# xiaoxiaokuye/CODLAD

Hardware: AMD Instinct MI355X
Metric: sampled all-atom structures/sec (100-step DDPM, PED) (higher is better)
Workload: dtype f32 as f16x3 split (each fp32 operand = fp16 hi + fp16 lo, 22-bit; 3 f16 MFMAs per product, fp32 accumulate); everything outside the contractions fp32; 1 GPU; cfg2: PED-shaped test set, 4 proteins L=46/87/92/129 x 10 frames x num_ensemble 10 = 400 structures per GPU, 100-step DDPM (mpnn_diffusion) + VQ(4096x3) + IC_Decoder N6 + ic_to_xyz; structures_rank0=400, nodes_rank0=35400, edges_rank0=2182800, ddpm_steps=100, parallelism=replicas x1

## Files before the change

### codlad_amd/_lib.py

```python
import ctypes as C
import os

import torch

_HERE = os.path.dirname(os.path.abspath(__file__))
ABI_VERSION = 15
LIB_PATH = os.environ.get("CODLAD_HIP_LIB") or os.path.join(_HERE, "libcodlad_hip.so")

P = C.c_void_p


class EncLayer(C.Structure):
    _fields_ = [(n, P) for n in ("W1e", "W2", "W3", "W11e", "W12", "W13", "W1a", "W1c", "W11a", "W11c")] + \
               [("Win", P * 4), ("Wout", P * 4)] + \
               [(n, P) for n in ("b1", "b2", "b3", "b11", "b12", "b13", "b_in", "b_out")]


class DecLayer(C.Structure):
    _fields_ = [(n, P) for n in ("W1e", "W2", "W3", "W1a", "W1v", "TS")] + \
               [("Win", P * 4), ("Wout", P * 4)] + \
               [(n, P) for n in ("b1", "b2", "b3", "b_in", "b_out")]


class EncLayerH(C.Structure):
    _fields_ = [(n, P) for n in ("W1e", "W2", "W3", "W11e", "W12", "W13", "W1a", "W1c", "W11a", "W11c")] + \
               [("Win", P * 4), ("Wout", P * 4)] + \
               [(n, P) for n in ("b1", "b2", "b3", "b11", "b12", "b13", "b_in", "b_out")] + \
               [(n, C.c_int) for n in ("e1", "e2", "e3", "e11", "e12", "e13", "e_in", "e_out")]


class DecLayerH(C.Structure):
    _fields_ = [(n, P) for n in ("W1e", "W2", "W3", "W1a", "W1v")] + [("Win", P * 4), ("Wout", P * 4)] + \
               [(n, P) for n in ("TS", "b1", "b2", "b3", "b_in", "b_out")] + \
               [(n, C.c_int) for n in ("e1", "e2", "e3", "e_in", "e_out")]


class DenoiserWeights(C.Structure):
    _fields_ = [(n, P) for n in ("freqs", "rbf_mu", "t_w0", "t_b0", "t_w2", "t_b2")] + \
               [("ada_w", P * 7), ("ada_b", P * 7)] + \
               [(n, P) for n in ("x_in_w", "x_in_b", "pos_w", "pos_b", "edge_wT", "norm_w", "norm_b",
                                 "We_wT", "We_b", "out_w", "out_b")] + \
               [("enc", EncLayer * 3), ("dec", DecLayer * 3), ("precision", C.c_int),
                ("enc_h", EncLayerH * 3), ("dec_h", DecLayerH * 3), ("self_condition", C.c_int), ("out_dim", C.c_int)]


class Workspace(C.Structure):
    _fields_ = [(n, P) for n in ("hV", "hVenc", "S", "PQ", "hE", "status", "tile_list")] + [("n_tiles", C.c_int32)]


class DecoderWeights(C.Structure):
    _fields_ = [("angle", C.c_int), ("map_out_w", P), ("map_out_b", P), ("res_embed", P)] + \
               [(n, P * 4) for n in ("inv0_w", "inv0_b", "inv1_w", "inv1_b", "dist_w", "dist_b",
                                     "dense1_w", "dense1_b", "dense3_w", "dense3_b")] + \
               [(n, P) for n in ("bb_dist", "sc_dist", "bb_ang1_w", "bb_ang1_b", "bb_ang3_w", "bb_ang3_b",
                                 "sc_angle_emb", "sc_ang1_w", "sc_ang1_b", "sc_ang3_w", "sc_ang3_b",
                                 "bb_tor1_w", "bb_tor1_b", "bb_tor3_w", "bb_tor3_b")] + \
               [(n, P * 4) for n in ("tor1_w", "tor1_b", "tor3_w", "tor3_b")] + \
               [(n, P) for n in ("fin1_w", "fin1_b", "fin3_w", "fin3_b")]


class TpConvArgs(C.Structure):
    _fields_ = [("ptr", P), ("snd", P), ("n_recv", C.c_int32), ("xyz_recv", P), ("xyz_snd", P), ("typ_recv", P),
                ("typ_snd", P), ("r_sign", C.c_float), ("smear_stop", C.c_float), ("emb0_w", P), ("emb0_b", P),
                ("emb3_w", P), ("emb3_b", P), ("emb_in", C.c_int32), ("h_recv", P), ("d_recv", C.c_int32), ("h_snd", P),
                ("d_snd", C.c_int32), ("attr_recv_first", C.c_int32), ("fc0_w", P), ("fc0_b", P), ("fc3_w", P),
                ("fc3_b", P), ("depth", C.c_int32), ("out", P), ("accumulate", C.c_int32), ("group", C.c_int32),
                ("packed", P)]


class XyzGroup(C.Structure):
    _fields_ = [("ca_full", P), ("ic", P), ("orders", P), ("slot_to_out", P), ("xyz_out", P),
                ("B", C.c_int32), ("L", C.c_int32), ("n_atoms", C.c_int32), ("first_row", C.c_int32)]


class MetricInputs(C.Structure):
    _fields_ = [("xyz_recon", P), ("xyz", P), ("n_atoms", C.c_int64),
                ("edge_list", P), ("n_edges", C.c_int64), ("clash_list", P), ("n_clash", C.c_int64),
                ("bb_NO_list", P), ("n_bb", C.c_int64), ("interaction_list", P), ("n_inter", C.c_int64),
                ("pi_pi_list", P), ("n_pipi", C.c_int64),
                ("ic", P), ("ic_recon", P), ("ic_mask", P), ("n_ic", C.c_int64)]


_SIGS = {
    "codlad_abi_version": (C.c_int, []),
    "codlad_probe_edge_launches": (C.c_int, [C.c_int]),
    "codlad_probe_read": (C.c_int, [C.c_int, C.POINTER(C.c_double)]),
    "codlad_metrics_scratch_bytes": (C.c_int, []),
    "codlad_eval_metrics": (C.c_int, [C.POINTER(MetricInputs), P, P, P]),
    "codlad_bond_graph_counts": (C.c_int, [P, P, P, P, P, C.c_int, C.c_int, C.c_float, P, P]),
    "codlad_last_error": (C.c_char_p, []),
    "codlad_struct_sizes": (None, [C.POINTER(C.c_int)]),
    "codlad_pack_block_host": (None, [P, C.c_int, C.c_float, P]),
    "codlad_features_prepass": (C.c_int, [C.POINTER(DenoiserWeights), P, P, C.c_int, C.c_int, P, P, P]),
    "codlad_step_mods": (C.c_int, [C.POINTER(DenoiserWeights), P, C.c_int, P, P]),
    "codlad_step_mods_f": (C.c_int, [C.POINTER(DenoiserWeights), P, C.c_int, P, P]),
    "codlad_ode_combine": (C.c_int, [P, P, P, C.c_int, C.c_float, C.c_size_t, P, P]),
    "codlad_layer0_edge_terms": (C.c_int, [C.POINTER(DenoiserWeights), P, C.c_int, P, P, P]),
    "codlad_denoiser_forward": (C.c_int, [C.POINTER(DenoiserWeights), P, C.c_int, P, P, P, C.c_int, P, P, P, P,
                                          C.POINTER(Workspace), P]),
    "codlad_status_check": (C.c_int, [P, P]),
    "codlad_set_option": (C.c_int, [C.c_int, C.c_int]),
    "codlad_ddpm_update": (C.c_int, [P, P, P, P, C.c_int, P, P, P]),
    "codlad_ddpm_pred_xstart": (C.c_int, [P, P, P, C.c_int, P, P]),
    "codlad_ddpm_posterior_step": (C.c_int, [P, P, P, P, P, P, C.c_float, C.c_int, P, P, P]),
    "codlad_sample_loop": (C.c_int, [C.POINTER(DenoiserWeights), P, C.c_int, P, P, P, C.c_int, P, P, P, P, P,
                                     C.c_int, C.POINTER(Workspace), P]),
    "codlad_sample_loop_pinned": (C.c_int, [C.POINTER(DenoiserWeights), P, C.c_int, P, P, P, C.c_int, P, P, P, P, P,
                                            C.c_int, P, P, C.POINTER(Workspace), P]),
    "codlad_ddim_loop": (C.c_int, [C.POINTER(DenoiserWeights), P, C.c_int, P, P, P, C.c_int, P, P, P, P, P, C.c_int,
                                   C.c_int, C.c_int, P, P, C.POINTER(Workspace), P]),
    "codlad_ddim_step": (C.c_int, [P, P, P, P, P, C.c_int, C.c_int, P, P, P]),
    "codlad_vq_lookup": (C.c_int, [P, C.c_int, P, P, P, C.c_int, P, P, P, P]),
    "codlad_ic_decode": (C.c_int, [C.POINTER(DecoderWeights), P, P, P, P, P, C.c_int, P, P, P]),
    "codlad_cg_graph": (C.c_int, [P, P, C.c_int, C.c_float, P, P, P, P]),
    "codlad_ic_to_xyz": (C.c_int, [P, P, P, P, C.c_int, C.c_int, C.c_int, P, P]),
    "codlad_ic_to_xyz_groups": (C.c_int, [P, C.c_int, C.c_int, P]),
    "codlad_xyz_to_ic": (C.c_int, [P, C.c_int, C.c_int, P, C.c_int, P, P]),
    "codlad_tp_conv_image_bytes": (C.c_int, [C.c_int]),
    "codlad_tp_conv_pack": (C.c_int, [P, P, P]),
    "codlad_receiver_csr": (C.c_int, [P, C.c_int, C.c_int, C.c_int, P, P, P, P]),
    "codlad_bench_edge_launch": (C.c_int, [C.POINTER(DenoiserWeights), P, C.c_int, P, P, P,
                                           C.POINTER(Workspace), C.c_int, C.c_int, P]),
    "codlad_tp_conv": (C.c_int, [C.POINTER(TpConvArgs), P]),
    "codlad_tp_conv_args_size": (C.c_int, []),
    "codlad_mlp_rows": (C.c_int, [P, C.c_int, C.c_int, P, P, C.c_int, P, P, C.c_int, C.c_int, C.c_int, P, P]),
    "codlad_bead_mean": (C.c_int, [P, P, P, P, C.c_int, P, P]),
    "codlad_embed_rows": (C.c_int, [P, P, C.c_int, C.c_int, P, P]),
    "codlad_selftest_gemm128": (C.c_int, [P, P, P, C.c_int, C.c_int, P, P]),
    "codlad_selftest_gemm128_h": (C.c_int, [P, P, P, C.c_int, C.c_int, C.c_int, P, P]),
}

_lib = None


def lib():
    global _lib
    if _lib is None:
        if not os.path.exists(LIB_PATH):
            raise RuntimeError(
                f"{LIB_PATH} is missing: the HIP extension is the only implementation of this path "
                "(build it with `python -m codlad_amd.build`)")
        handle = C.CDLL(LIB_PATH, mode=C.RTLD_GLOBAL)
        for name, (res, args) in _SIGS.items():
            fn = getattr(handle, name)
            fn.restype = res
            fn.argtypes = args
        if handle.codlad_abi_version() != ABI_VERSION:
            raise RuntimeError("libcodlad_hip.so ABI version mismatch")
        _lib = handle
    return _lib


OPT_NODEQ_MAX_TILES, OPT_EDGE_TILE_MAX_NODES, OPT_DEC_EDGE_VARIANT, OPT_TP_CONV_VARIANT, OPT_EDGE_UPD_VARIANT, OPT_EDGE_CUS, OPT_EDGE_WIDE_MAX_TILES, OPT_NODE_QUAD_MAX_TILES = 0, 1, 3, 4, 5, 6, 7, 2


def set_option(option, value):
    check(lib().codlad_set_option(option, value), "codlad_set_option")


def exported_symbols():
    return list(_SIGS)


def check(rc, what):
    if rc != 0:
        msg = lib().codlad_last_error().decode() or "unknown error"
        raise RuntimeError(f"{what} failed (rc={rc}): {msg}")


class _TensorPtr(C.c_void_p):
    """c_void_p that keeps its tensor alive for as long as the argument object lives, i.e. until
    the foreign call has been enqueued.  (A bare integer would let a temporary such as
    `x.contiguous()` be freed - and its block reused by the next temporary - before the launch.)"""


def ptr(t):
    if t is None:
        return None
    assert t.is_contiguous(), "non-contiguous tensor handed to the C ABI"
    p = _TensorPtr(t.data_ptr())
    p._keepalive = t
    return p


def stream_ptr(device=None):
    return C.c_void_p(torch.cuda.current_stream(device).cuda_stream)
```

### codlad_amd/csrc/denoiser_kernels.hip

```cpp
#include "common.h"
#include <stdlib.h>
#include "../../include/codlad_hip.h"

#include "edge_args.h"


template <bool EDGE_UPDATE>
__global__ __launch_bounds__(256, 2) void edge_kernel(EdgeArgs a) {
    const int lane = threadIdx.x & 63;
    const int n = blockIdx.x * 4 + (threadIdx.x >> 6);
    if (n >= a.n_nodes) return;
    const int h = lane >> 5, c = lane & 31;
    const int4 info = a.node_info[n];
    const int src = info.x, base = info.y, K = info.z;
    const float *rows = a.hE_in + (size_t)(a.in_by_src ? src : n) * (64 * HD);
    const float *Prow = a.P + (size_t)n * HD;

    for (int half = 0; half < 2; ++half) {
        if (32 * half >= K) break;
        const int col = 32 * half + c;
        const bool valid = col < K;
        const int colc = valid ? col : 0;
        const int j = a.E_idx[(size_t)src * 64 + colc];

        Tile x, acc;
        tile_load_row(acc, Prow, h);
        tile_add_row(acc, a.Q + (size_t)(base + j) * HD, h);
        if (a.E1) {
            tile_add_edge(acc, a.E1 + (size_t)src * EDGE_BLOCK, colc, h);
        } else {
            tile_load_edge(x, rows, colc, h);
            gemm128(acc, x, a.W1, lane);
        }
        const GeluK gk = gelu_consts(0);
        tile_gelu(acc, gk);
        tile_load_row(x, a.b2, h);
        gemm128(x, acc, a.W2, lane);
        tile_gelu(x, gk);

        if (!EDGE_UPDATE) {
            float *Srow = a.S + (size_t)n * HD;
#pragma unroll
            for (int bo = 0; bo < 4; ++bo)
#pragma unroll
                for (int r = 0; r < 16; ++r) {
                    x.b[bo][r] = half_wave_sum(valid ? x.b[bo][r] : 0.f);
                }
            if (c == 31) {
                if (half) tile_add_row(x, Srow, h);
                tile_store_row(x, Srow, h);
            }
        } else {
            tile_load_row(acc, a.b3, h);
            gemm128(acc, x, a.W3, lane);
            tile_add_edge(acc, rows, colc, h);
            tile_layernorm(acc, 1e-6f);
            tile_modulate(acc, a.mods3, a.mods3 + HD, a.mods3 + 2 * HD, h);
            if (valid) tile_store_edge(acc, a.hE_out + (size_t)n * EDGE_BLOCK, col, h);
        }
    }
}

#include "node_args.h"

template <bool MODE_UPD>
__global__ __launch_bounds__(64, 1) void node_kernel(NodeArgs a) {
    const int lane = threadIdx.x & 63;
    const int h = lane >> 5, c = lane & 31;
    const int node = blockIdx.x * 32 + c;
    const bool valid = node < a.n_nodes;
    const int nc = valid ? node : a.n_nodes - 1;
    const int4 info = a.node_info[nc];

    Tile v;
    if (!MODE_UPD) {
        const float x0 = a.x[nc * 3 + 0], x1 = a.x[nc * 3 + 1], x2 = a.x[nc * 3 + 2];
        const bool sc = a.in_dim == 6;
        const bool have_sc = sc && a.x_sc != nullptr;
        const float s0 = have_sc ? a.x_sc[nc * 3 + 0] : 0.f, s1 = have_sc ? a.x_sc[nc * 3 + 1] : 0.f,
                    s2 = have_sc ? a.x_sc[nc * 3 + 2] : 0.f;
        tile_load_row(v, a.x_in_b, h);
#pragma unroll
        for (int bo = 0; bo < 4; ++bo)
#pragma unroll
            for (int r = 0; r < 16; ++r) {
                const int f = 32 * bo + (r & 3) + 8 * (r >> 2) + 4 * h;
                const float *wr = a.x_in_w + f * a.in_dim;
                float acc = 0.f;
                if (sc) {
                    acc = fmaf(s2, wr[2], fmaf(s1, wr[1], s0 * wr[0]));
                    wr += 3;
                }
                v.b[bo][r] += fmaf(x2, wr[2], fmaf(x1, wr[1], fmaf(x0, wr[0], acc)));
            }
    } else {
        Tile s, t;
        tile_load_row(s, a.S + (size_t)nc * HD, h);
        tile_load_row(t, a.b3, h);
        const float kf = (float)info.z;
#pragma unroll
        for (int bo = 0; bo < 4; ++bo) t.b[bo] *= kf;
        gemm128(t, s, a.W3, lane);
        tile_load_row(v, a.hV + (size_t)nc * HD, h);
#pragma unroll
        for (int bo = 0; bo < 4; ++bo)
#pragma unroll
            for (int r = 0; r < 16; ++r) v.b[bo][r] += t.b[bo][r] / 30.0f;
        tile_layernorm(v, 1e-6f);
        tile_modulate(v, a.mods, a.mods + HD, a.mods + 2 * HD, h);
        tile_load_row(t, a.b_out, h);
#pragma unroll 1
        for (int ch = 0; ch < 4; ++ch) {
            tile_load_row(s, a.b_in + ch * HD, h);
            gemm128(s, v, a.Win[ch], lane);
            tile_gelu(s, gelu_consts(0));
            gemm128(t, s, a.Wout[ch], lane);
        }
#pragma unroll
        for (int bo = 0; bo < 4; ++bo) v.b[bo] += t.b[bo];
        tile_layernorm(v, 1e-6f);
        tile_modulate(v, a.mods + 3 * HD, a.mods + 4 * HD, a.mods + 5 * HD, h);
    }
    if (valid) {
        tile_store_row(v, a.hV + (size_t)node * HD, h);
        if (a.hVenc_out) tile_store_row(v, a.hVenc_out + (size_t)node * HD, h);
    }

#pragma unroll 1
    for (int p = 0; p < a.n_proj; ++p) {
        Tile in = v, out;
        const int fl = a.proj_flags[p];
        if (fl & 1) {
            if (a.venc_is_self) {
#pragma unroll
                for (int bo = 0; bo < 4; ++bo) in.b[bo] += v.b[bo];
            } else {
                tile_add_row(in, a.hVenc_in + (size_t)nc * HD, h);
            }
        }
        if (a.proj_b[p]) tile_load_row(out, a.proj_b[p], h);
        else tile_zero(out);
        if (fl & 2) tile_add_row(out, a.TS + (size_t)info.w * HD, h);
        gemm128(out, in, a.proj_w[p], lane);
        if (valid) tile_store_row(out, a.proj_out[p] + (size_t)node * HD, h);
    }
}

template <bool MODE_UPD, int NW, int TERMS>
__global__ __launch_bounds__(NW * 64, (NW + 3) / 4) void node_kernel_h(NodeArgs a) {
    extern __shared__ __align__(16) u32x4 wl[];
    constexpr int NT = NW * 64;
    constexpr int PER_T = LDS_BLOCK_U4 / NT;
    static_assert(LDS_BLOCK_U4 % NT == 0, "block must divide evenly over the workgroup");
    const int tid = threadIdx.x, lane = tid & 63, wave = tid >> 6;
    const int h = lane >> 5, c = lane & 31;
    const int wg_node0 = a.n_nodes >= XCD_CHUNKED_NODE_KERNEL_MIN
                             ? (blockIdx.x % 8) * xcd_chunk_nodes(a.n_nodes) + (blockIdx.x / 8) * (32 * NW)
                             : blockIdx.x * (32 * NW);
    if (wg_node0 >= a.n_nodes) return;
    const int node = wg_node0 + wave * 32 + c;
    const bool valid = node < a.n_nodes;
    const int nc = valid ? node : a.n_nodes - 1;
    const int4 info = a.node_info[nc];
    const int n_blk = (MODE_UPD ? 9 : 0) + a.n_proj;

    int cur = 0;
    auto fetch = [&](int i) {
        const u32x4 *g = reinterpret_cast<const u32x4 *>(a.blk_h[i]);
        u32x4 *dst = wl + (i & 1) * LDS_BLOCK_U4;
#pragma unroll
        for (int q = 0; q < PER_T; ++q) {
            const int chunk = (q * NW + wave) * 64;
            __builtin_amdgcn_global_load_lds(g + chunk + lane,
                                             (__attribute__((address_space(3))) void *)(dst + chunk), 16, 0, 0);
        }
    };
    auto landed = [&]() { __builtin_amdgcn_s_waitcnt(0x0F70); };
    auto apply = [&](Tile &acc, const Tile &in, bool gelu_in) {
        const bool more = cur + 1 < n_blk;
        if (more) fetch(cur + 1);
        const u32x4 *w = wl + (cur & 1) * LDS_BLOCK_U4;
        if (gelu_in) gemm128_h_lds<TERMS, true>(acc, in, w, lane, a.gelu_ffn);
        else gemm128_h_lds<TERMS, false>(acc, in, w, lane, a.gelu_ffn);
        if (more) landed();
        __syncthreads();
        ++cur;
    };
    if (n_blk > 0) {
        fetch(0);
        landed();
    }
    const float *modAB = reinterpret_cast<const float *>(wl + 2 * LDS_BLOCK_U4);
    if (MODE_UPD && tid < 64) {
        const float4 *m = reinterpret_cast<const float4 *>(a.mods) + 96 * (tid >> 5);
        const int i = tid & 31;
        const float4 s = m[i], c = m[32 + i], g = m[64 + i];
        float4 *cf = reinterpret_cast<float4 *>(wl + 2 * LDS_BLOCK_U4) + 64 * (tid >> 5);
        cf[i] = make_float4(g.x * (1.0f + c.x), g.y * (1.0f + c.y), g.z * (1.0f + c.z), g.w * (1.0f + c.w));
        cf[32 + i] = make_float4(g.x * s.x, g.y * s.y, g.z * s.z, g.w * s.w);
    }
    __syncthreads();

    Tile v;
    if (!MODE_UPD) {
        const float x0 = a.x[nc * 3 + 0], x1 = a.x[nc * 3 + 1], x2 = a.x[nc * 3 + 2];
        const bool sc = a.in_dim == 6;
        const bool have_sc = sc && a.x_sc != nullptr;
        const float s0 = have_sc ? a.x_sc[nc * 3 + 0] : 0.f, s1 = have_sc ? a.x_sc[nc * 3 + 1] : 0.f,
                    s2 = have_sc ? a.x_sc[nc * 3 + 2] : 0.f;
        tile_load_row(v, a.x_in_b, h);
#pragma unroll
        for (int bo = 0; bo < 4; ++bo)
#pragma unroll
            for (int r = 0; r < 16; ++r) {
                const int f = 32 * bo + (r & 3) + 8 * (r >> 2) + 4 * h;
                const float *wr = a.x_in_w + f * a.in_dim;
                float acc = 0.f;
                if (sc) {
                    acc = fmaf(s2, wr[2], fmaf(s1, wr[1], s0 * wr[0]));
                    wr += 3;
                }
                v.b[bo][r] += fmaf(x2, wr[2], fmaf(x1, wr[1], fmaf(x0, wr[0], acc)));
            }
    } else {
        Tile s, t;
        tile_load_row(s, a.S + (size_t)nc * HD, h);
        if (a.s_partials) {
            const size_t plane = (size_t)a.n_nodes * HD;
            tile_load_row(t, a.S + 2 * plane + (size_t)nc * HD, h);
            if (info.z > 32) {
                tile_add_row(s, a.S + plane + (size_t)nc * HD, h);
                tile_add_row(t, a.S + 3 * plane + (size_t)nc * HD, h);
            }
#pragma unroll
            for (int bo = 0; bo < 4; ++bo) s.b[bo] += t.b[bo];
        }
        tile_load_row(t, a.b3, h);
        const float kf = (float)info.z * 0.015625f;
#pragma unroll
        for (int bo = 0; bo < 4; ++bo) {
            t.b[bo] *= kf;
            s.b[bo] *= a.s_scale;
        }
        apply(t, s, false);
        tile_load_row(v, a.hV + (size_t)nc * HD, h);
#pragma unroll
        for (int bo = 0; bo < 4; ++bo)
#pragma unroll
            for (int r = 0; r < 16; ++r) v.b[bo][r] += (t.b[bo][r] * a.t_scale) / 30.0f;
        tile_layernorm_affine(v, 1e-6f, modAB, modAB + HD, h);
        tile_load_row(t, a.b_out, h);
#pragma unroll 1
        for (int ch = 0; ch < 4; ++ch) {
            tile_load_row(s, a.b_in + ch * HD, h);
            apply(s, v, false);
            apply(t, s, true);
        }
#pragma unroll
        for (int bo = 0; bo < 4; ++bo) v.b[bo] += t.b[bo] * a.ffn_scale;
        tile_layernorm_affine(v, 1e-6f, modAB + 2 * HD, modAB + 3 * HD, h);
    }
    if (valid) {
        tile_store_row(v, a.hV + (size_t)node * HD, h);
        if (a.hVenc_out) tile_store_row(v, a.hVenc_out + (size_t)node * HD, h);
    }
#pragma unroll 1
    for (int p = 0; p < a.n_proj; ++p) {
        Tile in = v, out;
        const int fl = a.proj_flags[p];
        if (fl & 1) {
            if (a.venc_is_self) {
#pragma unroll
                for (int bo = 0; bo < 4; ++bo) in.b[bo] += v.b[bo];
            } else {
                tile_add_row(in, a.hVenc_in + (size_t)nc * HD, h);
            }
        }
        if (a.proj_b[p]) tile_load_row(out, a.proj_b[p], h);
        else tile_zero(out);
        if (fl & 2) tile_add_row(out, a.TS + (size_t)info.w * HD, h);
        apply(out, in, false);
        if (valid) tile_store_row(out, a.proj_out[p] + (size_t)node * HD, h);
    }
}

struct FinalArgs {
    const float *hV;
    const float *mods;
    const float *out_w, *out_b;
    int n_nodes;
    float *logits;
    float *x;
    const float *noise;
    const float *coef;
    float *x_start;
    int *status;
    int n_out;
};

DEV float half_wave_allsum(float v) {
#pragma unroll
    for (int m = 16; m >= 1; m >>= 1) v += __shfl_xor(v, m, 64);
    return v;
}

#define CODLAD_STEP_DDPM 0
#define CODLAD_STEP_DDIM 1
#define CODLAD_STEP_DDIM_REVERSE 2
template <bool PIN, int STEP = CODLAD_STEP_DDPM>
__global__ __launch_bounds__(256) void final_kernel(FinalArgs a, const float *pin_x0, const uint8_t *pin_mask, int mode) {
    const int l = threadIdx.x & 31;
    const int n = blockIdx.x * 8 + (threadIdx.x >> 5);
    const bool live = n < a.n_nodes;
    const int nc = live ? n : a.n_nodes - 1;
    const float4 v = reinterpret_cast<const float4 *>(a.hV + (size_t)nc * HD)[l];
    const float mean = half_wave_allsum((v.x + v.y) + (v.z + v.w)) * (1.0f / 128.0f);
    const float d0 = v.x - mean, d1 = v.y - mean, d2 = v.z - mean, d3 = v.w - mean;
    const float var = half_wave_allsum((d0 * d0 + d1 * d1) + (d2 * d2 + d3 * d3));
    const float rstd = 1.0f / sqrtf(var * (1.0f / 128.0f) + 1e-6f);
    const float4 sh = reinterpret_cast<const float4 *>(a.mods)[l], sc = reinterpret_cast<const float4 *>(a.mods + HD)[l];
    const float m0 = (d0 * rstd) * (1.0f + sc.x) + sh.x, m1 = (d1 * rstd) * (1.0f + sc.y) + sh.y,
                m2 = (d2 * rstd) * (1.0f + sc.z) + sh.z, m3 = (d3 * rstd) * (1.0f + sc.w) + sh.w;
    float o[6];
#pragma unroll
    for (int k = 0; k < 6; ++k) {
        o[k] = 0.f;
        if (k < a.n_out) {
            const float4 w = reinterpret_cast<const float4 *>(a.out_w + k * HD)[l];
            o[k] = half_wave_allsum(fmaf(m3, w.w, fmaf(m2, w.z, fmaf(m1, w.y, m0 * w.x)))) + a.out_b[k];
        }
    }
    if (!live) return;
    if (a.status && l == 0) {
        bool bad = false;
#pragma unroll
        for (int k = 0; k < 6; ++k) {
            unsigned u = __float_as_uint(o[k]);
            asm volatile("" : "+v"(u));
            bad |= (u & 0x7f800000u) == 0x7f800000u;
        }
        if (bad) atomicOr(a.status, CODLAD_STATUS_NONFINITE);
    }
    if (a.logits) {
        if (l < a.n_out) {
            float mine = o[0];
#pragma unroll
            for (int k = 1; k < 6; ++k) mine = l == k ? o[k] : mine;
            a.logits[(size_t)n * a.n_out + l] = mine;
        }
        return;
    }
    if (l < 3) {
        const float eps = l == 0 ? o[0] : (l == 1 ? o[1] : o[2]);
        const float vv = l == 0 ? o[3] : (l == 1 ? o[4] : o[5]);
        const size_t i = (size_t)n * 3 + l;
        const float *pin = PIN && pin_mask[n] ? pin_x0 + i : nullptr;
        if constexpr (STEP == CODLAD_STEP_DDPM)
            a.x[i] = ddpm_step(a.x[i], eps, vv, a.coef, a.noise[i], a.x_start ? a.x_start + i : nullptr, pin);
        else if constexpr (STEP == CODLAD_STEP_DDIM)
            a.x[i] = ddim_step<false>(a.x[i], eps, a.coef, mode, a.noise[i], a.x_start ? a.x_start + i : nullptr, pin);
        else
            a.x[i] = ddim_step<true>(a.x[i], eps, a.coef, mode, 0.f, a.x_start ? a.x_start + i : nullptr, pin);
    }
}

struct DdpmCoef {
    float c[8];
};

__global__ void ddpm_kernel(const float *x, const float *out, const float *noise, DdpmCoef cf,
                            int n_nodes, float *x_out, float *x_start) {
    const int i = blockIdx.x * blockDim.x + threadIdx.x;
    if (i >= n_nodes * 3) return;
    const int n = i / 3, k = i - 3 * n;
    const bool fixed = ((int)cf.c[7] & CODLAD_DDPM_FIXED_VAR) != 0;
    const float o = fixed ? out[n * 3 + k] : out[n * 6 + k], v = fixed ? 0.f : out[n * 6 + 3 + k];
    x_out[i] = ddpm_step(x[i], o, v, cf.c, noise[i], x_start ? x_start + i : nullptr);
}

__global__ void ddpm_pred_xstart_kernel(const float *x, const float *out, DdpmCoef cf, int n_nodes, float *x0_out) {
    const int i = blockIdx.x * blockDim.x + threadIdx.x;
    if (i >= n_nodes * 3) return;
    const int n = i / 3, k = i - 3 * n;
    const bool fixed = ((int)cf.c[7] & CODLAD_DDPM_FIXED_VAR) != 0;
    x0_out[i] = ddpm_raw_x0(x[i], fixed ? out[n * 3 + k] : out[n * 6 + k], cf.c);
}

__global__ void ddpm_posterior_kernel(const float *x, const float *x0, const float *out, const float *noise,
                                      const float *grad, DdpmCoef cf, float fixed_variance, int n_nodes, float *x_out,
                                      float *x_start) {
    const int i = blockIdx.x * blockDim.x + threadIdx.x;
    if (i >= n_nodes * 3) return;
    const int n = i / 3, k = i - 3 * n;
    const bool fixed = ((int)cf.c[7] & CODLAD_DDPM_FIXED_VAR) != 0;
    const float logvar = ddpm_log_variance(fixed ? 0.f : out[n * 6 + 3 + k], cf.c);
    const float variance = fixed ? fixed_variance : expf(logvar);
    x_out[i] = ddpm_posterior(x[i], x0[i], logvar, cf.c, noise[i], x_start ? x_start + i : nullptr,
                              grad ? grad + i : nullptr, variance);
}

template <bool REVERSE>
__global__ void ddim_update_kernel(const float *x, const float *x0, const float *noise, const float *grad, DdpmCoef cf,
                                   int mode, int n_nodes, float *x_out, float *x_start) {
    const int i = blockIdx.x * blockDim.x + threadIdx.x;
    if (i >= n_nodes * 3) return;
    x_out[i] = ddim_update<REVERSE>(x[i], x0[i], cf.c, mode, REVERSE ? 0.f : noise[i], x_start ? x_start + i : nullptr,
                                    grad ? grad + i : nullptr);
}

__global__ __launch_bounds__(256) void mods_kernel(codlad_denoiser_weights w, const int64_t *tv, const float *tf,
                                                  float *mods) {
    __shared__ float emb[256];
    __shared__ float hid[HD];
    __shared__ float sc[HD];
    const int tid = threadIdx.x;
    const float t = tv ? (float)tv[blockIdx.x] : tf[blockIdx.x];
    {
        const int k = tid & 127;
        const float arg = t * w.freqs[k];
        emb[tid] = tid < 128 ? cosf(arg) : sinf(arg);
    }
    __syncthreads();
    if (tid < HD) {
        float acc = 0.f;
        const float *wr = w.t_w0 + tid * 256;
        for (int k = 0; k < 256; ++k) acc = fmaf(emb[k], wr[k], acc);
        acc += w.t_b0[tid];
        hid[tid] = acc / (1.0f + expf(-acc));
    }
    __syncthreads();
    if (tid < HD) {
        float acc = 0.f;
        const float *wr = w.t_w2 + tid * HD;
        for (int k = 0; k < HD; ++k) acc = fmaf(hid[k], wr[k], acc);
        acc += w.t_b2[tid];
        sc[tid] = acc / (1.0f + expf(-acc));
    }
    __syncthreads();
    float *out = mods + (size_t)blockIdx.x * CODLAD_MODS_PER_STEP;
    int off = 0;
    for (int hd = 0; hd < 7; ++hd) {
        const int rows = hd < 3 ? 9 * HD : (hd < 6 ? 6 * HD : 2 * HD);
        for (int r = tid; r < rows; r += 256) {
            const float *wr = w.ada_w[hd] + (size_t)r * HD;
            float acc = 0.f;
            for (int k = 0; k < HD; ++k) acc = fmaf(sc[k], wr[k], acc);
            out[off + r] = acc + w.ada_b[hd][r];
        }
        off += rows;
    }
}

static inline int mods_offset(int head) {
    return head < 3 ? head * 9 * HD : (head < 6 ? 27 * HD + (head - 3) * 6 * HD : 45 * HD);
}

static int g_num_cu = 0;

int num_cu() {
    if (!g_num_cu) {
        int dev = 0, n = 0;
        if (hipGetDevice(&dev) != hipSuccess ||
            hipDeviceGetAttribute(&n, hipDeviceAttributeMultiprocessorCount, dev) != hipSuccess || n <= 0)
            n = 256;
        g_num_cu = n;
    }
    return g_num_cu;
}

static hipError_t g_attr_error = hipSuccess;
void set_max_lds(const void *fn, size_t bytes) {
    const hipError_t e = hipFuncSetAttribute(fn, hipFuncAttributeMaxDynamicSharedMemorySize, (int)bytes);
    if (e != hipSuccess && g_attr_error == hipSuccess) g_attr_error = e;
}
hipError_t codlad_take_attr_error() {
    const hipError_t e = g_attr_error;
    g_attr_error = hipSuccess;
    return e;
}

void launch_edge_tile(int terms, bool update, const EdgeArgs &ea, const int2 *tile_list, int n_tiles, hipStream_t st);
void launch_edge_wide(int terms, bool update, const EdgeArgs &ea, const int2 *tile_list, int n_tiles, hipStream_t st);
int edge_wide_max_tiles();
void launch_edge_msg(int terms, const EdgeArgs &ea, hipStream_t st);
void launch_edge_upd(int terms, const EdgeArgs &ea, hipStream_t st);
void launch_edge_upd1(int terms, const EdgeArgs &ea, hipStream_t st);
int edge_upd_variant();

template <int TERMS>
static void launch_edge_h(bool update, const EdgeArgs &ea, const int2 *tile_list, int n_tiles, hipStream_t st) {
    if (tile_list && n_tiles <= edge_wide_max_tiles()) return launch_edge_wide(TERMS, update, ea, tile_list, n_tiles, st);
    if (tile_list) return launch_edge_tile(TERMS, update, ea, tile_list, n_tiles, st);
    if (update) {
        const bool two_tiles_each = n_tiles > 0 && 20ll * n_tiles >= 19ll * 2 * ea.n_nodes;
        if ((edge_upd_variant() == 1 && two_tiles_each) || edge_upd_variant() == 2) launch_edge_upd1(TERMS, ea, st);
        else launch_edge_upd(TERMS, ea, st);
    } else launch_edge_msg(TERMS, ea, st);
}

static void launch_edge_now(bool update, const EdgeArgs &ea, int precision, hipStream_t st, const int2 *tile_list,
                            int n_tiles) {
    if (precision == 2) return launch_edge_h<3>(update, ea, tile_list, n_tiles, st);
    if (precision == 1) return launch_edge_h<4>(update, ea, tile_list, n_tiles, st);
    dim3 grid((ea.n_nodes + 3) / 4), block(256);
    if (update) hipLaunchKernelGGL(edge_kernel<true>, grid, block, 0, st, ea);
    else hipLaunchKernelGGL(edge_kernel<false>, grid, block, 0, st, ea);
}

#define PROBE_MAX 4096
static struct {
    bool on = false;
    int used = 0;
    hipEvent_t ev[PROBE_MAX][2] = {};
    bool made[PROBE_MAX] = {};
    int kind[PROBE_MAX] = {};
} g_probe;

static void launch_edge(bool update, const EdgeArgs &ea, int precision, hipStream_t st, const int2 *tile_list = nullptr,
                        int n_tiles = 0) {
    const int i = g_probe.used;
    bool rec = g_probe.on && i < PROBE_MAX;
    if (rec && !g_probe.made[i]) {
        rec = hipEventCreate(&g_probe.ev[i][0]) == hipSuccess && hipEventCreate(&g_probe.ev[i][1]) == hipSuccess;
        g_probe.made[i] = rec;
    }
    if (rec) (void)hipEventRecord(g_probe.ev[i][0], st);
    launch_edge_now(update, ea, precision, st, tile_list, n_tiles);
    if (rec) {
        (void)hipEventRecord(g_probe.ev[i][1], st);
        g_probe.kind[i] = (update ? 1 : 0) + (ea.E1 ? 2 : 0);
        g_probe.used = i + 1;
    }
}

extern "C" int codlad_probe_edge_launches(int enable) {
    g_probe.on = enable != 0;
    if (enable) g_probe.used = 0;
    return 0;
}

extern "C" int codlad_probe_read(int kind, double *total_ms) {
    CODLAD_REQUIRE(total_ms && kind >= 0 && kind < 4, "bad arguments");
    double sum = 0.0;
    int n = 0;
    for (int i = 0; i < g_probe.used; ++i) {
        if (g_probe.kind[i] != kind) continue;
        float ms = 0.f;
        hipError_t e = hipEventSynchronize(g_probe.ev[i][1]);
        if (e == hipSuccess) e = hipEventElapsedTime(&ms, g_probe.ev[i][0], g_probe.ev[i][1]);
        if (e != hipSuccess) { codlad_set_error("codlad_probe_read: %s", hipGetErrorString(e)); return -(int)e - 1000; }
        sum += ms;
        ++n;
    }
    *total_ms = sum;
    return n;
}

template <int TERMS, int NW>
static void launch_node_hw(bool upd, const NodeArgs &na, hipStream_t st) {
    static bool attr_set = false;
    const size_t lds = 2 * 65536 + 4 * 512;
    if (!attr_set) {
        set_max_lds(reinterpret_cast<const void *>(node_kernel_h<true, NW, TERMS>), lds);
        set_max_lds(reinterpret_cast<const void *>(node_kernel_h<false, NW, TERMS>), lds);
        attr_set = true;
    }
    static_assert(NODE_WG_TILE % (32 * NW) == 0, "chunks hold whole workgroup tiles");
    const int wgs = na.n_nodes >= XCD_CHUNKED_NODE_KERNEL_MIN ? 8 * (xcd_chunk_nodes(na.n_nodes) / (32 * NW))
                                                              : (na.n_nodes + 32 * NW - 1) / (32 * NW);
    dim3 grid(wgs), block(NW * 64);
    if (upd) hipLaunchKernelGGL((node_kernel_h<true, NW, TERMS>), grid, block, lds, st, na);
    else hipLaunchKernelGGL((node_kernel_h<false, NW, TERMS>), grid, block, lds, st, na);
}

static int g_options[CODLAD_N_OPTIONS] = {-1, -1, -1, -1, -1, -1, -1, -1};
static int option_or(int opt, const char *env, int dflt) {
    if (g_options[opt] < 0) {
        const char *e = getenv(env);
        g_options[opt] = e ? atoi(e) : dflt;
    }
    return g_options[opt];
}
extern "C" int codlad_set_option(int option, int value) {
    CODLAD_REQUIRE(option >= 0 && option < CODLAD_N_OPTIONS && value >= 0, "unknown option or negative value");
    g_options[option] = value;
    return 0;
}
static int edge_tile_max_nodes() { return option_or(CODLAD_OPT_EDGE_TILE_MAX_NODES, "CODLAD_EDGE_TILE_MAX_NODES", 1 << 30); }
static int nodeq_max_tiles() { return option_or(CODLAD_OPT_NODEQ_MAX_TILES, "CODLAD_NODEQ_MAX_TILES", 256); }
int dec_edge_variant() { return option_or(CODLAD_OPT_DEC_EDGE_VARIANT, "CODLAD_DEC_EDGE_VARIANT", 0); }
int tp_conv_variant() { return option_or(CODLAD_OPT_TP_CONV_VARIANT, "CODLAD_TP_CONV_VARIANT", 0); }
int edge_upd_variant() { return option_or(CODLAD_OPT_EDGE_UPD_VARIANT, "CODLAD_EDGE_UPD_VARIANT", 0); }
int edge_wide_max_tiles() { return option_or(CODLAD_OPT_EDGE_WIDE_MAX_TILES, "CODLAD_EDGE_WIDE_MAX_TILES", 22 * num_cu()); }
int edge_cus() {
    const int v = option_or(CODLAD_OPT_EDGE_CUS, "CODLAD_EDGE_CUS", 0);
    return v > 0 && v < num_cu() ? v : num_cu();
}

void launch_node_wide(int terms, bool upd, const NodeArgs &na, hipStream_t st);
void launch_node_quad(int terms, const NodeArgs &na, hipStream_t st);
static int node_quad_max_tiles() { return option_or(CODLAD_OPT_NODE_QUAD_MAX_TILES, "CODLAD_NODE_QUAD_MAX_TILES", 2 * num_cu()); }

template <int TERMS>
static void launch_node_h(bool upd, const NodeArgs &na, hipStream_t st) {
    const int tiles = (na.n_nodes + 31) / 32;
    if (upd && tiles <= node_quad_max_tiles()) launch_node_quad(TERMS, na, st);
    else if (tiles <= nodeq_max_tiles()) launch_node_wide(TERMS, upd, na, st);
    else if (tiles > 4 * num_cu()) launch_node_hw<TERMS, 8>(upd, na, st);
    else launch_node_hw<TERMS, 4>(upd, na, st);
}

static void launch_node(bool upd, const NodeArgs &na, int precision, hipStream_t st) {
    if (precision == 2) return launch_node_h<3>(upd, na, st);
    if (precision == 1) return launch_node_h<4>(upd, na, st);
    dim3 grid((na.n_nodes + 31) / 32), block(64);
    if (upd) hipLaunchKernelGGL(node_kernel<true>, grid, block, 0, st, na);
    else hipLaunchKernelGGL(node_kernel<false>, grid, block, 0, st, na);
}

static void set_msg_scales(EdgeArgs &ea, bool split, const float *b2, const float *b2h, int e1, int e2) {
    ea.b2 = split ? b2h : b2;
    ea.gelu_a = gelu_consts(split ? e1 : 0);
    ea.gelu_b = gelu_consts(split ? e1 + e2 : 0);
    ea.res_scale = 1.0f; ea.ln_eps = 1e-6f;
}
static void set_upd_scales(EdgeArgs &eu, bool split, const codlad_enc_layer &L, const codlad_enc_layer_h &Lh) {
    eu.b2 = split ? Lh.b12 : L.b12; eu.b3 = split ? Lh.b13 : L.b13;
    const int E2 = split ? Lh.e11 + Lh.e12 : 0, E3 = split ? E2 + Lh.e13 : 0;
    eu.gelu_a = gelu_consts(split ? Lh.e11 : 0);
    eu.gelu_b = gelu_consts(E2);
    eu.res_scale = pow2i(E3);
    eu.ln_eps = 1e-6f * pow2i(2 * E3);
}
static void set_node_scales(NodeArgs &na, bool split, int e_msg, int e3, int e_in, int e_out) {
    na.s_scale = 0.015625f * pow2i(split ? -e_msg : 0);
    na.t_scale = 64.0f * pow2i(split ? -e3 : 0);
    na.ffn_scale = pow2i(split ? -(e_in + e_out) : 0);
    na.gelu_ffn = gelu_consts(split ? e_in : 0);
}

static void enqueue_forward(const codlad_denoiser_weights *w, const int32_t *node_info,
                            int n_nodes, const int32_t *E_idx, const float *h_E0, const float *E1,
                            size_t n_snodes, const float *x, const float *x_self_cond, const float *mods_t,
                            const codlad_workspace *ws, hipStream_t st) {
    const int4 *ni = reinterpret_cast<const int4 *>(node_info);
    const size_t NS = (size_t)n_nodes * HD;
    float *PQ0 = ws->PQ, *PQ1 = ws->PQ + NS, *PQ2 = ws->PQ + 2 * NS, *PQ3 = ws->PQ + 3 * NS;
    const bool split = w->precision != 0;
    const bool tilewise = split && ws->tile_list && ws->n_tiles > 0 &&
                          (ws->n_tiles <= 8 * num_cu() || ws->n_tiles <= edge_wide_max_tiles()) &&
                          n_nodes <= edge_tile_max_nodes();
    const int2 *tile_list = tilewise ? reinterpret_cast<const int2 *>(ws->tile_list) : nullptr;

    {
        NodeArgs na = {};
        na.node_info = ni; na.n_nodes = n_nodes;
        na.x = x; na.x_in_w = w->x_in_w; na.x_in_b = w->x_in_b; na.hV = ws->hV;
        na.x_sc = x_self_cond; na.in_dim = w->self_condition ? 6 : 3;
        na.n_proj = 2;
        na.proj_w[0] = w->enc[0].W1a; na.proj_b[0] = split ? w->enc_h[0].b1 : w->enc[0].b1; na.proj_out[0] = PQ0;
        na.proj_w[1] = w->enc[0].W1c; na.proj_b[1] = nullptr;      na.proj_out[1] = PQ1;
        na.blk_h[0] = w->enc_h[0].W1a; na.blk_h[1] = w->enc_h[0].W1c;
        set_node_scales(na, split, 0, 0, 0, 0);
        launch_node(false, na, w->precision, st);
    }
    for (int l = 0; l < 3; ++l) {
        const codlad_enc_layer &L = w->enc[l];
        const codlad_enc_layer_h &Lh = w->enc_h[l];
        const float *m = mods_t + mods_offset(l);
        EdgeArgs ea = {};
        ea.node_info = ni; ea.E_idx = E_idx; ea.n_nodes = n_nodes;
        ea.hE_in = l == 0 ? h_E0 : ws->hE; ea.in_by_src = l == 0;
        ea.P = PQ0; ea.Q = PQ1; ea.W1 = L.W1e; ea.W2 = L.W2; ea.S = ws->S;
        ea.W1h = Lh.W1e; ea.W2h = Lh.W2;
        set_msg_scales(ea, split, L.b2, Lh.b2, Lh.e1, Lh.e2);
        if (l == 0 && E1) ea.E1 = E1;
        launch_edge(false, ea, w->precision, st, tile_list, ws->n_tiles);

        NodeArgs na = {};
        na.node_info = ni; na.n_nodes = n_nodes; na.S = ws->S; na.hV = ws->hV;
        na.W3 = L.W3; na.b3 = split ? Lh.b3 : L.b3; na.mods = m;
        for (int c = 0; c < 4; ++c) { na.Win[c] = L.Win[c]; na.Wout[c] = L.Wout[c]; }
        na.b_in = split ? Lh.b_in : L.b_in; na.b_out = split ? Lh.b_out : L.b_out;
        set_node_scales(na, split, Lh.e1 + Lh.e2, Lh.e3, Lh.e_in, Lh.e_out);
        na.s_partials = tilewise;
        na.n_proj = 4;
        na.proj_w[0] = L.W11a; na.proj_b[0] = split ? Lh.b11 : L.b11; na.proj_out[0] = PQ2;
        na.proj_w[1] = L.W11c; na.proj_b[1] = nullptr;                 na.proj_out[1] = PQ3;
        if (l < 2) {
            na.proj_w[2] = w->enc[l + 1].W1a; na.proj_b[2] = split ? w->enc_h[l + 1].b1 : w->enc[l + 1].b1; na.proj_out[2] = PQ0;
            na.proj_w[3] = w->enc[l + 1].W1c; na.proj_b[3] = nullptr;          na.proj_out[3] = PQ1;
        } else {
            na.proj_w[2] = w->dec[0].W1a; na.proj_b[2] = split ? w->dec_h[0].b1 : w->dec[0].b1; na.proj_out[2] = PQ0;
            na.proj_w[3] = w->dec[0].W1v; na.proj_b[3] = nullptr;      na.proj_out[3] = PQ1;
            na.proj_flags[3] = 3; na.TS = split ? w->dec_h[0].TS : w->dec[0].TS;
            na.hVenc_out = ws->hVenc; na.venc_is_self = 1;
        }
        {
            int k = 0;
            na.blk_h[k++] = Lh.W3;
            for (int c = 0; c < 4; ++c) { na.blk_h[k++] = Lh.Win[c]; na.blk_h[k++] = Lh.Wout[c]; }
            na.blk_h[k++] = Lh.W11a; na.blk_h[k++] = Lh.W11c;
            if (l < 2) { na.blk_h[k++] = w->enc_h[l + 1].W1a; na.blk_h[k++] = w->enc_h[l + 1].W1c; }
            else { na.blk_h[k++] = w->dec_h[0].W1a; na.blk_h[k++] = w->dec_h[0].W1v; }
        }
        launch_node(true, na, w->precision, st);

        EdgeArgs eu = {};
        eu.node_info = ni; eu.E_idx = E_idx; eu.n_nodes = n_nodes;
        eu.hE_in = l == 0 ? h_E0 : ws->hE; eu.in_by_src = l == 0; eu.hE_out = ws->hE;
        eu.P = PQ2; eu.Q = PQ3; eu.W1 = L.W11e; eu.W2 = L.W12; eu.W3 = L.W13;
        eu.mods3 = m + 6 * HD;
        eu.W1h = Lh.W11e; eu.W2h = Lh.W12; eu.W3h = Lh.W13;
        set_upd_scales(eu, split, L, Lh);
        if (l == 0 && E1) eu.E1 = E1 + n_snodes * 64 * HD;
        launch_edge(true, eu, w->precision, st, tile_list, ws->n_tiles);
    }
    for (int l = 0; l < 3; ++l) {
        const codlad_dec_layer &L = w->dec[l];
        const codlad_dec_layer_h &Lh = w->dec_h[l];
        EdgeArgs ea = {};
        ea.node_info = ni; ea.E_idx = E_idx; ea.n_nodes = n_nodes;
        ea.hE_in = ws->hE; ea.in_by_src = 0;
        ea.P = PQ0; ea.Q = PQ1; ea.W1 = L.W1e; ea.W2 = L.W2; ea.S = ws->S;
        ea.W1h = Lh.W1e; ea.W2h = Lh.W2;
        set_msg_scales(ea, split, L.b2, Lh.b2, Lh.e1, Lh.e2);
        launch_edge(false, ea, w->precision, st, tile_list, ws->n_tiles);

        NodeArgs na = {};
        na.node_info = ni; na.n_nodes = n_nodes; na.S = ws->S; na.hV = ws->hV; na.s_partials = tilewise;
        na.W3 = L.W3; na.b3 = split ? Lh.b3 : L.b3; na.mods = mods_t + mods_offset(3 + l);
        for (int c = 0; c < 4; ++c) { na.Win[c] = L.Win[c]; na.Wout[c] = L.Wout[c]; }
        na.b_in = split ? Lh.b_in : L.b_in; na.b_out = split ? Lh.b_out : L.b_out;
        set_node_scales(na, split, Lh.e1 + Lh.e2, Lh.e3, Lh.e_in, Lh.e_out);
        if (l < 2) {
            na.n_proj = 2;
            na.proj_w[0] = w->dec[l + 1].W1a; na.proj_b[0] = split ? w->dec_h[l + 1].b1 : w->dec[l + 1].b1; na.proj_out[0] = PQ0;
            na.proj_w[1] = w->dec[l + 1].W1v; na.proj_b[1] = nullptr;          na.proj_out[1] = PQ1;
            na.proj_flags[1] = 3; na.TS = split ? w->dec_h[l + 1].TS : w->dec[l + 1].TS; na.hVenc_in = ws->hVenc;
        }
        {
            int k = 0;
            na.blk_h[k++] = Lh.W3;
            for (int c = 0; c < 4; ++c) { na.blk_h[k++] = Lh.Win[c]; na.blk_h[k++] = Lh.Wout[c]; }
            if (l < 2) { na.blk_h[k++] = w->dec_h[l + 1].W1a; na.blk_h[k++] = w->dec_h[l + 1].W1v; }
        }
        launch_node(true, na, w->precision, st);
    }
}

static int check_ws(const codlad_workspace *ws) {
    return ws && ws->hV && ws->hVenc && ws->S && ws->PQ && ws->hE;
}

extern "C" int codlad_step_mods(const codlad_denoiser_weights *w, const int64_t *t_values, int n_t,
                                float *mods, void *stream) {
    CODLAD_REQUIRE(w && t_values && mods, "null pointer");
    CODLAD_REQUIRE(n_t > 0, "n_t must be positive");
    hipLaunchKernelGGL(mods_kernel, dim3(n_t), dim3(256), 0, (hipStream_t)stream, *w, t_values, (const float *)nullptr, mods);
    return codlad_check_launch("codlad_step_mods");
}

extern "C" int codlad_step_mods_f(const codlad_denoiser_weights *w, const float *t_values, int n_t, float *mods,
                                  void *stream) {
    CODLAD_REQUIRE(w && t_values && mods, "null pointer");
    CODLAD_REQUIRE(n_t > 0, "n_t must be positive");
    hipLaunchKernelGGL(mods_kernel, dim3(n_t), dim3(256), 0, (hipStream_t)stream, *w, (const int64_t *)nullptr, t_values, mods);
    return codlad_check_launch("codlad_step_mods_f");
}


extern "C" int codlad_denoiser_forward(const codlad_denoiser_weights *w, const int32_t *node_info,
                                       int n_nodes, const int32_t *E_idx, const float *h_E0,
                                       const float *E1, int n_snodes, const float *x,
                                       const float *x_self_cond, const float *mods_t, float *out,
                                       const codlad_workspace *ws, void *stream) {
    CODLAD_REQUIRE(w && node_info && E_idx && h_E0 && x && mods_t && out, "null pointer");
    CODLAD_REQUIRE(check_ws(ws), "incomplete workspace");
    CODLAD_REQUIRE(n_nodes > 0, "n_nodes must be positive");
    hipStream_t st = (hipStream_t)stream;
    CODLAD_REQUIRE(!x_self_cond || w->self_condition, "x_self_cond given to a model without self-conditioning");
    CODLAD_REQUIRE(w->out_dim == 6 || w->out_dim == 3, "out_dim must be 6 (diffusion) or 3 (flow matching)");
    enqueue_forward(w, node_info, n_nodes, E_idx, h_E0, E1, (size_t)n_snodes, x, x_self_cond, mods_t, ws, st);
    FinalArgs fa = {};
    fa.hV = ws->hV; fa.mods = mods_t + mods_offset(6); fa.out_w = w->out_w; fa.out_b = w->out_b;
    fa.n_nodes = n_nodes; fa.logits = out; fa.status = ws->status; fa.n_out = w->out_dim;
    hipLaunchKernelGGL(final_kernel<false>, dim3((n_nodes + 7) / 8), dim3(256), 0, st, fa, nullptr, nullptr, 0);
    return codlad_check_launch("codlad_denoiser_forward");
}

extern "C" int codlad_ddpm_update(const float *x, const float *model_out, const float *noise,
                                  const float *coef_host, int n_nodes, float *x_out, float *x_start_out,
                                  void *stream) {
    CODLAD_REQUIRE(x && model_out && noise && coef_host && x_out, "null pointer");
    CODLAD_REQUIRE(n_nodes > 0, "n_nodes must be positive");
    DdpmCoef cf;
    for (int k = 0; k < 8; ++k) cf.c[k] = coef_host[k];
    hipLaunchKernelGGL(ddpm_kernel, dim3((n_nodes * 3 + 255) / 256), dim3(256), 0,
                       (hipStream_t)stream, x, model_out, noise, cf, n_nodes, x_out, x_start_out);
    return codlad_check_launch("codlad_ddpm_update");
}

extern "C" int codlad_ddpm_pred_xstart(const float *x, const float *model_out, const float *coef_host, int n_nodes,
                                      float *pred_xstart, void *stream) {
    CODLAD_REQUIRE(x && model_out && coef_host && pred_xstart, "null pointer");
    CODLAD_REQUIRE(n_nodes > 0, "n_nodes must be positive");
    DdpmCoef cf;
    for (int k = 0; k < 8; ++k) cf.c[k] = coef_host[k];
    hipLaunchKernelGGL(ddpm_pred_xstart_kernel, dim3((n_nodes * 3 + 255) / 256), dim3(256), 0, (hipStream_t)stream, x,
                       model_out, cf, n_nodes, pred_xstart);
    return codlad_check_launch("codlad_ddpm_pred_xstart");
}

extern "C" int codlad_ddpm_posterior_step(const float *x, const float *pred_xstart, const float *model_out,
                                          const float *noise, const float *grad, const float *coef_host,
                                          float fixed_variance, int n_nodes, float *x_out, float *x_start_out,
                                          void *stream) {
    CODLAD_REQUIRE(x && pred_xstart && model_out && noise && coef_host && x_out, "null pointer");
    CODLAD_REQUIRE(n_nodes > 0, "n_nodes must be positive");
    DdpmCoef cf;
    for (int k = 0; k < 8; ++k) cf.c[k] = coef_host[k];
    hipLaunchKernelGGL(ddpm_posterior_kernel, dim3((n_nodes * 3 + 255) / 256), dim3(256), 0, (hipStream_t)stream, x,
                       pred_xstart, model_out, noise, grad, cf, fixed_variance, n_nodes, x_out, x_start_out);
    return codlad_check_launch("codlad_ddpm_posterior_step");
}

static int sample_loop(const codlad_denoiser_weights *w, const int32_t *node_info, int n_nodes, const int32_t *E_idx,
                       const float *h_E0, const float *E1, int n_snodes, float *x, float *x_start, const float *noise,
                       const float *mods, const float *coef, int T, const float *pin_x0, const uint8_t *pin_mask,
                       const codlad_workspace *ws, void *stream, int step = CODLAD_STEP_DDPM, int mode = 0) {
    hipStream_t st = (hipStream_t)stream;
    const bool sc = w->self_condition != 0;
    const bool reverse = step == CODLAD_STEP_DDIM_REVERSE;
    for (int k = 0; k < T; ++k) {
        const int i = reverse ? k : T - 1 - k;
        const float *mods_t = mods + (size_t)i * CODLAD_MODS_PER_STEP;
        enqueue_forward(w, node_info, n_nodes, E_idx, h_E0, E1, (size_t)n_snodes, x, sc && k > 0 ? x_start : nullptr,
                        mods_t, ws, st);
        FinalArgs fa = {};
        fa.hV = ws->hV; fa.mods = mods_t + mods_offset(6); fa.out_w = w->out_w; fa.out_b = w->out_b;
        fa.n_nodes = n_nodes; fa.x = x; fa.noise = reverse ? nullptr : noise + (size_t)k * n_nodes * 3;
        fa.coef = coef + (size_t)i * 8; fa.x_start = x_start; fa.status = ws->status; fa.n_out = w->out_dim;
        const dim3 grid((n_nodes + 7) / 8);
        if (step == CODLAD_STEP_DDIM) {
            if (pin_x0)
                hipLaunchKernelGGL((final_kernel<true, CODLAD_STEP_DDIM>), grid, dim3(256), 0, st, fa, pin_x0, pin_mask, mode);
            else
                hipLaunchKernelGGL((final_kernel<false, CODLAD_STEP_DDIM>), grid, dim3(256), 0, st, fa, nullptr, nullptr, mode);
        } else if (reverse) {
            if (pin_x0)
                hipLaunchKernelGGL((final_kernel<true, CODLAD_STEP_DDIM_REVERSE>), grid, dim3(256), 0, st, fa, pin_x0,
                                   pin_mask, mode);
            else
                hipLaunchKernelGGL((final_kernel<false, CODLAD_STEP_DDIM_REVERSE>), grid, dim3(256), 0, st, fa, nullptr,
                                   nullptr, mode);
        } else if (pin_x0) {
            hipLaunchKernelGGL(final_kernel<true>, dim3((n_nodes + 7) / 8), dim3(256), 0, st, fa, pin_x0, pin_mask, 0);
        } else {
            hipLaunchKernelGGL(final_kernel<false>, dim3((n_nodes + 7) / 8), dim3(256), 0, st, fa, nullptr, nullptr, 0);
        }
    }
    return 0;
}

#define SAMPLE_LOOP_REQUIRE()                                                                                          \
    CODLAD_REQUIRE(w && node_info && E_idx && h_E0 && x && noise && mods && coef, "null pointer");                     \
    CODLAD_REQUIRE(check_ws(ws), "incomplete workspace");                                                             \
    CODLAD_REQUIRE(n_nodes > 0 && T > 0, "n_nodes and T must be positive");                                           \
    CODLAD_REQUIRE(!w->self_condition || x_start, "a self-conditioned model needs the x_start buffer");               \
    CODLAD_REQUIRE(w->out_dim == 6 || w->out_dim == 3,                                                                \
                   "the DDPM loop needs a model with 6 outputs (mean | variance logits) or 3 (fixed-variance samplers)")

extern "C" int codlad_sample_loop(const codlad_denoiser_weights *w, const int32_t *node_info,
                                  int n_nodes, const int32_t *E_idx, const float *h_E0,
                                  const float *E1, int n_snodes, float *x, float *x_start,
                                  const float *noise, const float *mods, const float *coef, int T,
                                  const codlad_workspace *ws, void *stream) {
    SAMPLE_LOOP_REQUIRE();
    sample_loop(w, node_info, n_nodes, E_idx, h_E0, E1, n_snodes, x, x_start, noise, mods, coef, T, nullptr, nullptr, ws,
                stream);
    return codlad_check_launch("codlad_sample_loop");
}

extern "C" int codlad_sample_loop_pinned(const codlad_denoiser_weights *w, const int32_t *node_info,
                                         int n_nodes, const int32_t *E_idx, const float *h_E0,
                                         const float *E1, int n_snodes, float *x, float *x_start,
                                         const float *noise, const float *mods, const float *coef, int T,
                                         const float *pin_x0, const uint8_t *pin_mask,
                                         const codlad_workspace *ws, void *stream) {
    SAMPLE_LOOP_REQUIRE();
    CODLAD_REQUIRE(pin_x0 && pin_mask, "null pointer (pin_x0 / pin_mask)");
    sample_loop(w, node_info, n_nodes, E_idx, h_E0, E1, n_snodes, x, x_start, noise, mods, coef, T, pin_x0, pin_mask, ws,
                stream);
    return codlad_check_launch("codlad_sample_loop_pinned");
}
#undef SAMPLE_LOOP_REQUIRE

extern "C" int codlad_ddim_loop(const codlad_denoiser_weights *w, const int32_t *node_info, int n_nodes,
                                const int32_t *E_idx, const float *h_E0, const float *E1, int n_snodes, float *x,
                                float *x_start, const float *noise, const float *mods, const float *coef, int T, int mode,
                                int reverse, const float *pin_x0, const uint8_t *pin_mask, const codlad_workspace *ws,
                                void *stream) {
    CODLAD_REQUIRE(w && node_info && E_idx && h_E0 && x && mods && coef, "null pointer");
    CODLAD_REQUIRE(reverse || noise, "null pointer (noise: only the reverse loop runs without it)");
    CODLAD_REQUIRE(!pin_x0 == !pin_mask, "null pointer (pin_x0 and pin_mask come together)");
    CODLAD_REQUIRE(n_nodes > 0 && T > 0, "n_nodes and T must be positive");
    CODLAD_REQUIRE(mode >= 0 && mode <= (CODLAD_DDPM_START_X | CODLAD_DDPM_FIXED_VAR | CODLAD_DDPM_CLIP),
                   "unknown mode bits");
    CODLAD_REQUIRE(w->out_dim == ((mode & CODLAD_DDPM_FIXED_VAR) ? 3 : 6),
                   "mode and model disagree: a learned-range sampler needs a model with 6 outputs (mean | variance "
                   "logits), a fixed-variance one (mode bit 2) a model with 3");
    CODLAD_REQUIRE(!w->self_condition || x_start, "a self-conditioned model needs the x_start buffer");
    CODLAD_REQUIRE(check_ws(ws), "incomplete workspace");
    sample_loop(w, node_info, n_nodes, E_idx, h_E0, E1, n_snodes, x, x_start, noise, mods, coef, T, pin_x0, pin_mask, ws,
                stream, reverse ? CODLAD_STEP_DDIM_REVERSE : CODLAD_STEP_DDIM, mode);
    return codlad_check_launch("codlad_ddim_loop");
}

extern "C" int codlad_ddim_step(const float *x, const float *pred_xstart, const float *noise, const float *grad,
                                const float *coef_host, int reverse, int n_nodes, float *x_out, float *x_start_out,
                                void *stream) {
    CODLAD_REQUIRE(x && pred_xstart && coef_host && x_out, "null pointer");
    CODLAD_REQUIRE(reverse || noise, "null pointer (noise: only the reverse step runs without it)");
    CODLAD_REQUIRE(n_nodes > 0, "n_nodes must be positive");
    DdpmCoef cf;
    for (int k = 0; k < 8; ++k) cf.c[k] = coef_host[k];
    const int mode = (int)coef_host[7];
    const dim3 grid((n_nodes * 3 + 255) / 256);
    if (reverse)
        hipLaunchKernelGGL(ddim_update_kernel<true>, grid, dim3(256), 0, (hipStream_t)stream, x, pred_xstart, nullptr,
                           grad, cf, mode, n_nodes, x_out, x_start_out);
    else
        hipLaunchKernelGGL(ddim_update_kernel<false>, grid, dim3(256), 0, (hipStream_t)stream, x, pred_xstart, noise,
                           grad, cf, mode, n_nodes, x_out, x_start_out);
    return codlad_check_launch("codlad_ddim_step");
}

extern "C" int codlad_status_check(int32_t *status, void *stream) {
    CODLAD_REQUIRE(status, "null pointer");
    int32_t host = 0;
    hipStream_t st = (hipStream_t)stream;
    hipError_t e = hipMemcpyAsync(&host, status, sizeof(host), hipMemcpyDeviceToHost, st);
    if (e == hipSuccess) e = hipStreamSynchronize(st);
    if (e == hipSuccess && host) e = hipMemsetAsync(status, 0, sizeof(host), st);
    if (e != hipSuccess) {
        codlad_set_error("codlad_status_check: %s", hipGetErrorString(e));
        return (int)e;
    }
    if (host & CODLAD_STATUS_NONFINITE) {
        codlad_set_error("denoiser output is not finite: an input, a weight or - in the split-fp16 contraction "
                         "modes - an operand beyond the fp16 range (|x| > 65504) overflowed; rerun with precision f32 to tell them apart");
        return CODLAD_E_NONFINITE;
    }
    return 0;
}

struct Layer0Args {
    const int2 *snode_info;
    const float *hE0;
    const float *W_msg, *W_upd;
    const void *Wh_msg, *Wh_upd;
    float *E1;
    int n_snodes;
};

template <int TERMS>
__global__ __launch_bounds__(256, 1) void layer0_kernel(Layer0Args a) {
    const int lane = threadIdx.x & 63, h = lane >> 5, c = lane & 31;
    const int m = blockIdx.x * 4 + (threadIdx.x >> 6);
    if (m >= a.n_snodes) return;
    const int L = a.snode_info[m].y, K = L < 64 ? L : 64;
    for (int half = 0; half < 2; ++half) {
        if (32 * half >= K) break;
        const int col = 32 * half + c;
        const bool valid = col < K;
        const int colc = valid ? col : 0;
        Tile x;
        tile_load_edge(x, a.hE0 + (size_t)m * EDGE_BLOCK, colc, h);
#pragma unroll 1
        for (int which = 0; which < 2; ++which) {
            Tile acc;
            tile_zero(acc);
            if constexpr (TERMS != 0) gemm_h_glb<TERMS, 0, 8, false, true>(acc, x, which ? a.Wh_upd : a.Wh_msg, lane, gelu_consts(0));
            else gemm128(acc, x, which ? a.W_upd : a.W_msg, lane);
            if (valid) tile_store_edge(acc, a.E1 + ((size_t)which * a.n_snodes + m) * EDGE_BLOCK, col, h);
        }
    }
}

extern "C" int codlad_layer0_edge_terms(const codlad_denoiser_weights *w, const int32_t *snode_info,
                                        int n_snodes, const float *h_E0, float *E1, void *stream) {
    CODLAD_REQUIRE(w && snode_info && h_E0 && E1 && n_snodes > 0, "bad arguments");
    Layer0Args a = {};
    a.snode_info = reinterpret_cast<const int2 *>(snode_info); a.hE0 = h_E0; a.E1 = E1; a.n_snodes = n_snodes;
    a.W_msg = w->enc[0].W1e; a.W_upd = w->enc[0].W11e;
    a.Wh_msg = w->enc_h[0].W1e; a.Wh_upd = w->enc_h[0].W11e;
    dim3 grid((n_snodes + 3) / 4), block(256);
    if (w->precision == 2) hipLaunchKernelGGL(layer0_kernel<3>, grid, block, 0, (hipStream_t)stream, a);
    else if (w->precision == 1) hipLaunchKernelGGL(layer0_kernel<4>, grid, block, 0, (hipStream_t)stream, a);
    else hipLaunchKernelGGL(layer0_kernel<0>, grid, block, 0, (hipStream_t)stream, a);
    return codlad_check_launch("codlad_layer0_edge_terms");
}

extern "C" int codlad_bench_edge_launch(const codlad_denoiser_weights *w, const int32_t *node_info,
                                        int n_nodes, const int32_t *E_idx, const float *h_E0,
                                        const float *mods_t, const codlad_workspace *ws, int which,
                                        int layer, void *stream) {
    CODLAD_REQUIRE(w && node_info && E_idx && h_E0 && mods_t, "null pointer");
    CODLAD_REQUIRE(check_ws(ws), "incomplete workspace");
    CODLAD_REQUIRE(n_nodes > 0 && (which == 0 || which == 1) && (layer == 0 || layer == 1), "bad arguments");
    const size_t NS = (size_t)n_nodes * HD;
    const codlad_enc_layer &L = w->enc[layer];
    EdgeArgs ea = {};
    ea.node_info = reinterpret_cast<const int4 *>(node_info); ea.E_idx = E_idx; ea.n_nodes = n_nodes;
    ea.hE_in = layer == 0 ? h_E0 : ws->hE; ea.in_by_src = layer == 0;
    const codlad_enc_layer_h &Lh = w->enc_h[layer];
    const bool split = w->precision != 0;
    if (which == 0) {
        ea.P = ws->PQ; ea.Q = ws->PQ + NS; ea.W1 = L.W1e; ea.W2 = L.W2; ea.S = ws->S;
        ea.W1h = Lh.W1e; ea.W2h = Lh.W2;
        set_msg_scales(ea, split, L.b2, Lh.b2, Lh.e1, Lh.e2);
    } else {
        ea.hE_out = ws->hE; ea.P = ws->PQ + 2 * NS; ea.Q = ws->PQ + 3 * NS;
        ea.S = ws->S;
        ea.W1 = L.W11e; ea.W2 = L.W12; ea.W3 = L.W13;
        ea.mods3 = mods_t + 6 * HD;
        ea.W1h = Lh.W11e; ea.W2h = Lh.W12; ea.W3h = Lh.W13;
        set_upd_scales(ea, split, L, Lh);
    }
    launch_edge(which == 1, ea, w->precision, (hipStream_t)stream, nullptr, ws->n_tiles);
    return codlad_check_launch("codlad_bench_edge_launch");
}

__global__ __launch_bounds__(64) void selftest_kernel(const float *Wp, const float *bias,
                                                      const float *X, int n_rows, int act, float *Y) {
    const int lane = threadIdx.x, h = lane >> 5, c = lane & 31;
    const int row = blockIdx.x * 32 + c;
    const int rc = row < n_rows ? row : n_rows - 1;
    Tile in, acc;
    tile_load_row(in, X + (size_t)rc * HD, h);
    tile_load_row(acc, bias, h);
    gemm128(acc, in, Wp, lane);
    if (act) tile_gelu(acc, gelu_consts(0));
    if (row < n_rows) tile_store_row(acc, Y + (size_t)row * HD, h);
}

template <int TERMS>
__global__ __launch_bounds__(64) void selftest_h_kernel(const void *Wh, const float *bias, const float *X,
                                                        int n_rows, int act, float *Y) {
    const int lane = threadIdx.x, h = lane >> 5, c = lane & 31;
    const int row = blockIdx.x * 32 + c;
    const int rc = row < n_rows ? row : n_rows - 1;
    Tile in, acc;
    tile_load_row(in, X + (size_t)rc * HD, h);
    tile_load_row(acc, bias, h);
    if (act) gemm_h_glb<TERMS, 0, 8, true>(acc, in, Wh, lane, gelu_consts(0));
    else gemm_h_glb<TERMS, 0, 8, false>(acc, in, Wh, lane, gelu_consts(0));
    if (row < n_rows) tile_store_row(acc, Y + (size_t)row * HD, h);
}

extern "C" int codlad_selftest_gemm128_h(const void *W_split, const float *bias, const float *X, int n_rows,
                                         int act_in, int terms, float *Y, void *stream) {
    CODLAD_REQUIRE(W_split && bias && X && Y && n_rows > 0 && (terms == 3 || terms == 4), "bad arguments");
    dim3 grid((n_rows + 31) / 32), block(64);
    if (terms == 3) hipLaunchKernelGGL(selftest_h_kernel<3>, grid, block, 0, (hipStream_t)stream, W_split, bias, X, n_rows, act_in, Y);
    else hipLaunchKernelGGL(selftest_h_kernel<4>, grid, block, 0, (hipStream_t)stream, W_split, bias, X, n_rows, act_in, Y);
    return codlad_check_launch("codlad_selftest_gemm128_h");
}

extern "C" int codlad_selftest_gemm128(const float *W_packed, const float *bias, const float *X,
                                       int n_rows, int act, float *Y, void *stream) {
    CODLAD_REQUIRE(W_packed && bias && X && Y && n_rows > 0, "bad arguments");
    hipLaunchKernelGGL(selftest_kernel, dim3((n_rows + 31) / 32), dim3(64), 0, (hipStream_t)stream,
                       W_packed, bias, X, n_rows, act, Y);
    return codlad_check_launch("codlad_selftest_gemm128");
}
```

### codlad_amd/csrc/edge_args.h

```cpp
#pragma once
#include "common.h"
#include "../../include/codlad_hip.h"

#define HD 128

void set_max_lds(const void *fn, size_t bytes);
int num_cu();
int edge_cus();

struct EdgeArgs {
    const int4 *node_info;
    const int32_t *E_idx;
    const float *hE_in;
    int in_by_src;
    const float *E1;
    float *hE_out;
    const float *P, *Q;
    const float *W1, *W2, *W3;
    const void *W1h, *W2h, *W3h;
    const float *b2, *b3;
    const float *mods3;
    float *S;
    int n_nodes;
    GeluK gelu_a, gelu_b;
    float res_scale, ln_eps;
};

struct EdgeTileArgs : EdgeArgs {
    const int2 *tile_list;
    int n_tiles;
};

#define LDS_BLOCK_U4 4096

constexpr int NODE_WG_TILE = 256;
constexpr int XCD_CHUNKED_NODE_KERNEL_MIN = 32768;
__host__ __device__ inline int xcd_chunk_nodes(int n_nodes) {
    const int g = n_nodes >= XCD_CHUNKED_NODE_KERNEL_MIN ? NODE_WG_TILE : 32;
    const int tiles = (n_nodes + g - 1) / g;
    return g * ((tiles + 7) / 8);
}

struct NodeSpan {
    int first, end, stride;
};
DEV NodeSpan wave_node_span(int n_nodes, int nwaves, int wave) {
    const int nb = gridDim.x, b = blockIdx.x;
    if (nb % 8) return {b * nwaves + wave, n_nodes, nb * nwaves};
    const int chunk = xcd_chunk_nodes(n_nodes);
    const int lo = (b % 8) * chunk, hi = lo + chunk < n_nodes ? lo + chunk : n_nodes;
    return {lo + (b / 8) * nwaves + wave, hi, (nb / 8) * nwaves};
}

constexpr int UPD_W1_KS = 3;
constexpr int EDGE_CONST_U4 = 4 * 32;
template <bool EDGE_UPDATE, int NWAVES>
constexpr int edge_lds_u4() {
    return 2 * LDS_BLOCK_U4 + (EDGE_UPDATE ? UPD_W1_KS * 512 : 0) + EDGE_CONST_U4 + NWAVES * 32;
}
```

### codlad_amd/csrc/edge_msg_kernel.hip

```cpp
#include "edge_args.h"

template <int NWAVES, bool HOISTED, int TERMS>
__global__ __launch_bounds__(NWAVES * 64, NWAVES / 4) void msg_kernel_h(EdgeArgs a) {
    extern __shared__ __align__(16) u32x4 wl[];
    constexpr int NT = NWAVES * 64;
    const int tid = threadIdx.x, lane = tid & 63, wave = tid >> 6;
    u32x4 *consts = wl + 2 * LDS_BLOCK_U4;
    {
        const u32x4 *g1 = reinterpret_cast<const u32x4 *>(a.W1h);
        const u32x4 *g2 = reinterpret_cast<const u32x4 *>(a.W2h);
        for (int i = tid; i < LDS_BLOCK_U4; i += NT) {
            if (!HOISTED) wl[i] = g1[i];
            wl[LDS_BLOCK_U4 + i] = g2[i];
        }
        if (tid < 32) consts[tid] = reinterpret_cast<const u32x4 *>(a.b2)[tid];
        u32x4 *rep = consts + EDGE_CONST_U4 + NWAVES * 32;
        if (tid < 128) {
            const unsigned bv = reinterpret_cast<const unsigned *>(a.b2)[tid];
            for (int q = 0; q < 4; ++q) rep[q * 128 + tid] = u32x4{bv, bv, bv, bv};
        }
    }
    __syncthreads();
    const u32x4 *w1 = wl, *w2 = wl + LDS_BLOCK_U4;
    const float *c_b2 = reinterpret_cast<const float *>(consts);
    float2 *Pslot = reinterpret_cast<float2 *>(consts + EDGE_CONST_U4 + wave * 32);
    const int h = lane >> 5, c = lane & 31;
    const NodeSpan span = wave_node_span(a.n_nodes, NWAVES, wave);
    const int stride = span.stride, n_end = span.end;
    int n = span.first;
    if (n >= n_end) return;

    const float *xsrc = HOISTED ? a.E1 : a.hE_in;
    auto block_of = [&](int node, int s) {
        return xsrc + (size_t)((HOISTED || a.in_by_src) ? s : node) * EDGE_BLOCK;
    };
    const float2 *Prows = reinterpret_cast<const float2 *>(a.P);

    int4 info = a.node_info[n];
    int src = __builtin_amdgcn_readfirstlane(info.x), base = __builtin_amdgcn_readfirstlane(info.y);
    int K = __builtin_amdgcn_readfirstlane(info.z);
    int jA = a.E_idx[(size_t)src * 64 + (c < K ? c : 0)];
    int jB = a.E_idx[(size_t)src * 64 + (32 + c < K ? 32 + c : 0)];
    Pslot[lane] = Prows[(size_t)n * 64 + lane];
    int half = 0;
    Tile x, acc, t2;
    tile_load_edge<!HOISTED>(x, block_of(n, src), c < K ? c : 0, h);
    tile_load_row(acc, a.Q + (size_t)(base + jA) * HD, h);
    float sum[4] = {0.f, 0.f, 0.f, 0.f};
    const float4 *bias_rep = reinterpret_cast<const float4 *>(consts + EDGE_CONST_U4 + NWAVES * 32) + c;

    int4 ninfo = info;
    int nsrc = src, nbase = base, nK = K, njA = jA, njB = jB;
    float2 npv = {0.f, 0.f};
    for (;;) {
        const int n2 = n + stride;
        const bool next_node = n2 < n_end;
        const bool first_half = half == 0;
        if (first_half && next_node) ninfo = a.node_info[n2];
        tile_add_row(acc, reinterpret_cast<const float *>(Pslot), h);
        if (HOISTED) {
#pragma unroll
            for (int bo = 0; bo < 4; ++bo) acc.b[bo] += x.b[bo];
        } else {
            gemm128_h_lds<TERMS, false, false, true>(acc, x, w1, lane, a.gelu_a);
        }
        if (first_half && next_node) {
            nsrc = __builtin_amdgcn_readfirstlane(ninfo.x);
            nbase = __builtin_amdgcn_readfirstlane(ninfo.y);
            nK = __builtin_amdgcn_readfirstlane(ninfo.z);
            njA = a.E_idx[(size_t)nsrc * 64 + (c < nK ? c : 0)];
            njB = a.E_idx[(size_t)nsrc * 64 + (32 + c < nK ? 32 + c : 0)];
            npv = Prows[(size_t)n2 * 64 + lane];
        }
        const bool next_half = first_half && K > 32;
        {
            int rep_off = 0;
            asm volatile("" : "+v"(rep_off));
            const float4 *br = bias_rep + rep_off;
#pragma unroll
            for (int bo = 0; bo < 4; ++bo)
#pragma unroll
                for (int q = 0; q < 4; ++q) {
                    const float4 bv = br[q * 128 + 32 * bo];
                    t2.b[bo][4 * q + 0] = bv.x; t2.b[bo][4 * q + 1] = bv.y;
                    t2.b[bo][4 * q + 2] = bv.z; t2.b[bo][4 * q + 3] = bv.w;
                }
        }
        gemm128_h_lds<TERMS, true, true>(t2, acc, w2, lane, a.gelu_a);
        {
            const int pn = next_half ? n : (next_node ? n2 : n), ps = next_half ? src : nsrc;
            const int pe = next_half ? (32 + c < K ? 32 + c : 0) : (c < nK ? c : 0);
            const int pq = next_half ? base + jB : nbase + njA;
            tile_load_edge<!HOISTED>(x, block_of(pn, ps), pe, h);
            tile_load_row(acc, a.Q + (size_t)pq * HD, h);
            __builtin_amdgcn_sched_barrier(0);
        }
        tile_gelu(t2, a.gelu_b);
        const int cnt = K - 32 * half;
        if (cnt >= 32) {
#pragma unroll
            for (int bo = 0; bo < 4; ++bo) {
                f32x2 s2 = tile_pair(t2.b[bo], 0);
#pragma unroll
                for (int r = 2; r < 16; r += 2) s2 += tile_pair(t2.b[bo], r);
                sum[bo] += s2.x + s2.y;
            }
        } else {
#pragma unroll
            for (int bo = 0; bo < 4; ++bo) {
                float s0 = 0.f;
#pragma unroll
                for (int r = 0; r < 16; ++r) s0 += ((r & 3) + 8 * (r >> 2) + 4 * h < cnt) ? t2.b[bo][r] : 0.f;
                sum[bo] += s0;
            }
        }
        if (next_half) {
            half = 1;
            continue;
        }
#pragma unroll
        for (int bo = 0; bo < 4; ++bo) {
            const float tot = sum[bo] + __shfl_xor(sum[bo], 32);
            if (h == 0) a.S[(size_t)n * HD + 32 * bo + c] = tot;
            sum[bo] = 0.f;
        }
        if (!next_node) break;
        n = n2; src = nsrc; base = nbase; K = nK; jA = njA; jB = njB;
        Pslot[lane] = npv;
        half = 0;
    }
}


template <int TERMS>
static void launch_msg_t(const EdgeArgs &ea, hipStream_t st) {
    static bool attr_set = false;
    constexpr int NW = 8;
    const size_t lds = 16 * (edge_lds_u4<false, NW>() + 4 * 128);
    static_assert(16 * (edge_lds_u4<false, NW>() + 4 * 128) <= 160 * 1024, "kernel exceeds the CU's LDS");
    if (!attr_set) {
        set_max_lds(reinterpret_cast<const void *>(msg_kernel_h<NW, false, TERMS>), lds);
        set_max_lds(reinterpret_cast<const void *>(msg_kernel_h<NW, true, TERMS>), lds);
        attr_set = true;
    }
    const int groups = (ea.n_nodes + NW - 1) / NW;
    dim3 grid(groups < edge_cus() ? groups : edge_cus()), block(NW * 64);
    if (ea.E1 != nullptr) hipLaunchKernelGGL((msg_kernel_h<NW, true, TERMS>), grid, block, lds, st, ea);
    else hipLaunchKernelGGL((msg_kernel_h<NW, false, TERMS>), grid, block, lds, st, ea);
}

void launch_edge_msg(int terms, const EdgeArgs &ea, hipStream_t st) {
    if (terms == 3) launch_msg_t<3>(ea, st);
    else launch_msg_t<4>(ea, st);
}
```

### codlad_amd/csrc/edge_upd_kernel.hip

```cpp
#include "edge_args.h"

template <int NWAVES, bool HOISTED, int TERMS>
__global__ __launch_bounds__(NWAVES * 64, NWAVES / 4) void upd_kernel_h(EdgeArgs a) {
    extern __shared__ __align__(16) u32x4 wl[];
    constexpr int NT = NWAVES * 64;
    constexpr int W1_U4 = UPD_W1_KS * 512;
    const int tid = threadIdx.x, lane = tid & 63, wave = tid >> 6;
    u32x4 *consts = wl + 2 * LDS_BLOCK_U4 + W1_U4;
    {
        const u32x4 *g1 = reinterpret_cast<const u32x4 *>(a.W1h);
        const u32x4 *g2 = reinterpret_cast<const u32x4 *>(a.W2h);
        const u32x4 *g3 = reinterpret_cast<const u32x4 *>(a.W3h);
        for (int i = tid; i < LDS_BLOCK_U4; i += NT) {
            wl[i] = g2[i];
            wl[LDS_BLOCK_U4 + i] = g3[i];
        }
        if (!HOISTED)
            for (int i = tid; i < W1_U4; i += NT) wl[2 * LDS_BLOCK_U4 + i] = g1[i];
        if (tid < 32) consts[tid] = reinterpret_cast<const u32x4 *>(a.b2)[tid];
        if (tid >= 64 && tid < 96) consts[32 + (tid & 31)] = reinterpret_cast<const u32x4 *>(a.b3)[tid & 31];
        if (tid >= 128 && tid < 160) {
            const float4 *m = reinterpret_cast<const float4 *>(a.mods3);
            const int i = tid & 31;
            const float4 s = m[i], c = m[32 + i], g = m[64 + i];
            float4 *cf = reinterpret_cast<float4 *>(consts);
            cf[64 + i] = make_float4(g.x * (1.0f + c.x), g.y * (1.0f + c.y), g.z * (1.0f + c.z), g.w * (1.0f + c.w));
            cf[96 + i] = make_float4(g.x * s.x, g.y * s.y, g.z * s.z, g.w * s.w);
        }
    }
    __syncthreads();
    const u32x4 *w2 = wl, *w3 = wl + LDS_BLOCK_U4, *w1 = wl + 2 * LDS_BLOCK_U4;
    const float *c_base = reinterpret_cast<const float *>(consts);
    float *Pslot = reinterpret_cast<float *>(consts + EDGE_CONST_U4 + wave * 32);
    const int h = lane >> 5, c = lane & 31;
    const NodeSpan span = wave_node_span(a.n_nodes, NWAVES, wave);
    for (int n = span.first; n < span.end; n += span.stride) {
        const int4 info = a.node_info[n];
        const int src = info.x, base = info.y, K = info.z;
        const float *rows = a.hE_in + (size_t)(a.in_by_src ? src : n) * EDGE_BLOCK;
        float *out_rows = a.hE_out + (size_t)n * EDGE_BLOCK;
        const bool validA = c < K, validB = 32 + c < K;
        const int colA = validA ? c : 0, colB = validB ? 32 + c : 0;
        const int jA = a.E_idx[(size_t)src * 64 + colA], jB = a.E_idx[(size_t)src * 64 + colB];
        reinterpret_cast<float2 *>(Pslot)[lane] = reinterpret_cast<const float2 *>(a.P + (size_t)n * HD)[lane];

        for (int half = 0; half < 2; ++half) {
            if (32 * half >= K) break;
            const bool valid = half ? validB : validA;
            const int colc = half ? colB : colA, col = 32 * half + c;
            const int j = half ? jB : jA;
            Tile x, acc, t2;
            StreamedGemm<TERMS, UPD_W1_KS, 8 - UPD_W1_KS, false, 8, true> tail1;
            if (!HOISTED) tail1.start(a.W1h, lane);
            int lds_off = 0;
            asm volatile("" : "+v"(lds_off));
            const float *c_b2 = c_base + lds_off, *c_b3 = c_b2 + HD;
            const float *c_modA = c_b2 + 2 * HD, *c_modB = c_b2 + 3 * HD;
            tile_load_row(acc, a.Q + (size_t)(base + j) * HD, h);
            tile_add_row(acc, Pslot, h);
            if (!HOISTED) tile_load_edge<true>(x, rows, colc, h);
            if (HOISTED) {
                tile_add_edge(acc, a.E1 + (size_t)src * EDGE_BLOCK, colc, h);
                __builtin_amdgcn_sched_barrier(0);
                tile_load_edge<false>(x, rows, colc, h);
            } else {
                gemm_h_lds<TERMS, 0, UPD_W1_KS, false, false, true>(acc, x, w1, lane, a.gelu_a);
                tail1.run(acc, x, lane, a.gelu_a);
            }
            tile_load_row(t2, c_b2, h);
            gemm128_h_lds<TERMS, true>(t2, acc, w2, lane, a.gelu_a);
            tile_unsplit_scale_add_row(x, a.res_scale, c_b3, h);
            gemm128_h_lds<TERMS, true>(x, t2, w3, lane, a.gelu_b);
            tile_layernorm_affine(x, a.ln_eps, c_modA, c_modB, h);
            tile_presplit(x);
            if (valid) tile_store_edge<true>(x, out_rows, col, h);
        }
    }
}


template <int TERMS>
static void launch_upd_t(const EdgeArgs &ea, hipStream_t st) {
    static bool attr_set = false;
    constexpr int NW = 8;
    const size_t lds = 16 * edge_lds_u4<true, NW>();
    static_assert(16 * edge_lds_u4<true, NW>() <= 160 * 1024, "kernel exceeds the CU's LDS");
    if (!attr_set) {
        set_max_lds(reinterpret_cast<const void *>(upd_kernel_h<NW, false, TERMS>), lds);
        set_max_lds(reinterpret_cast<const void *>(upd_kernel_h<NW, true, TERMS>), lds);
        attr_set = true;
    }
    const int groups = (ea.n_nodes + NW - 1) / NW;
    dim3 grid(groups < edge_cus() ? groups : edge_cus()), block(NW * 64);
    if (ea.E1 != nullptr) hipLaunchKernelGGL((upd_kernel_h<NW, true, TERMS>), grid, block, lds, st, ea);
    else hipLaunchKernelGGL((upd_kernel_h<NW, false, TERMS>), grid, block, lds, st, ea);
}

void launch_edge_upd(int terms, const EdgeArgs &ea, hipStream_t st) {
    if (terms == 3) launch_upd_t<3>(ea, st);
    else launch_upd_t<4>(ea, st);
}
```

### codlad_amd/engine.py

```python
import ctypes as C
import os

import numpy as np
import torch

from . import _lib
from .weights import DEFAULT_PRECISION, DenoiserWeights, DecoderWeights

H = 128
KNN = 64
MODS = 6016


def _require_cuda(t, what):
    if not t.is_cuda:
        raise RuntimeError(f"{what} must live on the GPU: this path has no CPU implementation")


def edge_rows(blocks, split=False):
    lead = blocks.shape[:-4]
    if not split:
        return blocks.permute(*range(len(lead)), -4, -2, -3, -1).reshape(*lead, 64, -1)
    hv = blocks.contiguous().view(torch.float16).view(*lead, 2, 4, 2, 2, 2, 32, 8)
    val = hv[..., 0, :, :, :].float() + hv[..., 1, :, :, :].float()
    n = len(lead)
    val = val.permute(*range(n), n, n + 4, n + 1, n + 2, n + 3, n + 5)
    out = torch.empty(*lead, 2, 32, 4, 2, 16, dtype=torch.float32, device=blocks.device)
    for h in range(2):
        out[..., 4 * h:4 * h + 4] = val[..., h, 0:4]
        out[..., 8 + 4 * h:8 + 4 * h + 4] = val[..., h, 4:8]
    return out.reshape(*lead, 64, 128)


class Structures:

    def __init__(self, xyz_list, z_list, device):
        self.lens = [int(x.shape[0]) for x in xyz_list]
        assert all(L >= 1 for L in self.lens)
        self.offsets = np.concatenate([[0], np.cumsum(self.lens)]).astype(np.int64)
        self.n_snodes = int(self.offsets[-1])
        self.xyz = torch.cat([x.reshape(-1, 3).float() for x in xyz_list]).contiguous().to(device)
        self.z = torch.cat([z.reshape(-1).to(torch.int32) for z in z_list]).contiguous().to(device)
        info = np.empty((self.n_snodes, 2), dtype=np.int32)
        for f, L in enumerate(self.lens):
            info[self.offsets[f]:self.offsets[f + 1], 0] = self.offsets[f]
            info[self.offsets[f]:self.offsets[f + 1], 1] = L
        self.snode_info = torch.from_numpy(info).to(device)
        self.E_idx = None
        self.h_E0 = None
        self.E1 = None
        self.features_tag = None


class Job:

    def __init__(self, structures, sample_struct, device, edge_state=None):
        st = structures
        self.structures = st
        self.device = device
        self._parts = {}
        self.sample_struct = [int(s) for s in sample_struct]
        lens = [st.lens[f] for f in self.sample_struct]
        self.sample_lens = lens
        self.sample_off = np.concatenate([[0], np.cumsum(lens)]).astype(np.int64)
        self.n_nodes = int(self.sample_off[-1])
        info = np.empty((self.n_nodes, 4), dtype=np.int32)
        z_host = st.z.cpu().numpy()
        for s, f in enumerate(self.sample_struct):
            a, b = self.sample_off[s], self.sample_off[s + 1]
            L = lens[s]
            info[a:b, 0] = np.arange(st.offsets[f], st.offsets[f] + L)
            info[a:b, 1] = a
            info[a:b, 2] = min(KNN, L)
            info[a:b, 3] = z_host[st.offsets[f]:st.offsets[f] + L]
        assert info[:, 3].min() >= 0 and info[:, 3].max() < 30, "residue type outside W_s vocabulary"
        self.node_info = torch.from_numpy(info).to(device)
        n = self.n_nodes
        f32 = dict(dtype=torch.float32, device=device)
        self.hV = torch.empty(n, H, **f32)
        self.hVenc = torch.empty(n, H, **f32)
        self.S = torch.empty(4, n, H, **f32)
        self.PQ = torch.empty(4, n, H, **f32)
        self.hE = torch.empty(n, KNN, H, **f32) if edge_state is None else edge_state
        assert tuple(self.hE.shape) == (n, KNN, H) and self.hE.is_contiguous()
        self.status = torch.zeros(1, dtype=torch.int32, device=device)
        halves = np.where(info[:, 2] > 32, 2, 1)
        tiles = np.empty((int(halves.sum()), 2), dtype=np.int32)
        tiles[:, 0] = np.repeat(np.arange(n, dtype=np.int32), halves)
        first = np.cumsum(halves) - halves
        tiles[:, 1] = np.arange(tiles.shape[0], dtype=np.int32) - np.repeat(first, halves).astype(np.int32)
        self.tile_list = torch.from_numpy(tiles).to(device)
        ws = _lib.Workspace()
        ws.hV, ws.hVenc, ws.S, ws.PQ, ws.hE, ws.status, ws.tile_list = (
            _lib.ptr(t) for t in (self.hV, self.hVenc, self.S, self.PQ, self.hE, self.status, self.tile_list))
        ws.n_tiles = tiles.shape[0]
        self.ws = ws

    def workspace_bytes(self):
        return 4 * (self.hV.numel() * 2 + self.S.numel() + self.PQ.numel() + self.hE.numel())

    def parts(self, k=2):
        if k not in self._parts:
            subs, start = [], 0
            for p in range(k):
                members = list(range(p, len(self.sample_struct), k))
                n = int(sum(self.sample_lens[m] for m in members))
                sub = Job(self.structures, [self.sample_struct[m] for m in members], self.device,
                          edge_state=self.hE[start:start + n])
                idx = np.concatenate([np.arange(self.sample_off[m], self.sample_off[m + 1]) for m in members])
                subs.append((sub, torch.from_numpy(idx).to(self.device)))
                start += n
            self._parts[k] = subs
        return self._parts[k]


class Denoiser:

    def __init__(self, state_dict, device, precision=DEFAULT_PRECISION, block_exponents=True, self_condition=False,
                 out_dim=6):
        self.device = torch.device(device)
        if self.device.type != "cuda":
            raise RuntimeError("codlad_amd runs on an MI355X only; no CPU path exists")
        self.lib = _lib.lib()
        if state_dict is None:
            self.weights = DenoiserWeights.empty(self.device, self_condition, out_dim, precision)
        else:
            self.weights = DenoiserWeights(state_dict, self.device, precision, block_exponents=block_exponents)
        self._mods_cache = {}
        self._mods_generation = self.weights.generation

    def new_structures(self, xyz_list, z_list, hoist_layer0=True):
        st = Structures(xyz_list, z_list, self.device)
        st.E_idx = torch.empty(st.n_snodes, KNN, dtype=torch.int32, device=self.device)
        st.h_E0 = torch.empty(st.n_snodes, 2, H // 4, KNN // 2, 4, dtype=torch.float32, device=self.device)
        if hoist_layer0:
            st.E1 = torch.empty(2, st.n_snodes, 2, H // 4, KNN // 2, 4, dtype=torch.float32, device=self.device)
        return st

    def compute_features(self, st):
        rc = self.lib.codlad_features_prepass(C.byref(self.weights.struct), _lib.ptr(st.xyz),
                                              _lib.ptr(st.snode_info), st.n_snodes, max(st.lens),
                                              _lib.ptr(st.E_idx), _lib.ptr(st.h_E0),
                                              _lib.stream_ptr(self.device))
        _lib.check(rc, "codlad_features_prepass")
        if st.E1 is not None:
            rc = self.lib.codlad_layer0_edge_terms(C.byref(self.weights.struct), _lib.ptr(st.snode_info),
                                                   st.n_snodes, _lib.ptr(st.h_E0), _lib.ptr(st.E1),
                                                   _lib.stream_ptr(self.device))
            _lib.check(rc, "codlad_layer0_edge_terms")
        st.features_tag = self.features_tag()
        return st

    @property
    def split_edge_state(self):
        return self.weights.precision != "f32"

    def features_tag(self):
        if self.weights.precision == "f32":
            return ("f32", self.weights.generation)
        ex = self.weights.exponents["enc0"]
        return ("split", self.weights.precision, ex["e1"], ex["e11"], self.weights.generation)

    def _fresh_features(self, st):
        if st.features_tag != self.features_tag():
            self.compute_features(st)

    def prepare_structures(self, xyz_list, z_list, hoist_layer0=True):
        return self.compute_features(self.new_structures(xyz_list, z_list, hoist_layer0))

    def make_job(self, structures, sample_struct):
        return Job(structures, sample_struct, self.device)

    def step_mods(self, t_values, refresh=False):
        fractional = any(float(t) != int(t) for t in t_values)
        key = tuple(float(t) for t in t_values) if fractional else tuple(int(t) for t in t_values)
        if self._mods_generation != self.weights.generation:
            self._mods_cache.clear()
            self._mods_generation = self.weights.generation
        if refresh or key not in self._mods_cache:
            mods = torch.empty(len(key), MODS, dtype=torch.float32, device=self.device)
            if fractional:
                tv = torch.tensor(key, dtype=torch.float32, device=self.device)
                rc = self.lib.codlad_step_mods_f(C.byref(self.weights.struct), _lib.ptr(tv), len(key),
                                                 _lib.ptr(mods), _lib.stream_ptr(self.device))
            else:
                tv = torch.tensor(key, dtype=torch.int64, device=self.device)
                rc = self.lib.codlad_step_mods(C.byref(self.weights.struct), _lib.ptr(tv), len(key),
                                               _lib.ptr(mods), _lib.stream_ptr(self.device))
            _lib.check(rc, "codlad_step_mods")
            if len(self._mods_cache) > 64:
                self._mods_cache.clear()
            self._mods_cache[key] = mods
        return self._mods_cache[key]

    @property
    def self_condition(self):
        return self.weights.self_condition

    def check_status(self, job):
        _lib.check(self.lib.codlad_status_check(_lib.ptr(job.status), _lib.stream_ptr(self.device)),
                   "codlad_status_check")

    def forward(self, job, x, t_value, x_self_cond=None, check=True):
        _require_cuda(x, "x")
        x = x.contiguous().float()
        assert x.shape == (job.n_nodes, 3)
        if x_self_cond is not None:
            if not self.self_condition:
                raise ValueError("x_self_cond given to a model built without self_condition")
            _require_cuda(x_self_cond, "x_self_cond")
            x_self_cond = x_self_cond.contiguous().float()
            assert x_self_cond.shape == x.shape
        mods = self.step_mods([t_value])
        out = torch.empty(job.n_nodes, self.weights.out_dim, dtype=torch.float32, device=self.device)
        st = job.structures
        self._fresh_features(st)
        rc = self.lib.codlad_denoiser_forward(C.byref(self.weights.struct), _lib.ptr(job.node_info),
                                              job.n_nodes, _lib.ptr(st.E_idx), _lib.ptr(st.h_E0),
                                              _lib.ptr(st.E1), st.n_snodes, _lib.ptr(x), _lib.ptr(x_self_cond),
                                              _lib.ptr(mods), _lib.ptr(out), C.byref(job.ws),
                                              _lib.stream_ptr(self.device))
        _lib.check(rc, "codlad_denoiser_forward")
        if check:
            self.check_status(job)
        return out

    SPLIT_MIN_NODES = int(os.environ.get("CODLAD_SAMPLE_SPLIT_MIN_NODES", 8192))

    SAMPLE_KINDS = ("ddpm", "ddim", "ddim_reverse")

    def sample(self, job, x_T, noise, tables, check=True, coef=None, streams=None, pin=None, kind="ddpm"):
        if kind not in self.SAMPLE_KINDS:
            raise ValueError(f"kind must be one of {self.SAMPLE_KINDS}, got {kind!r}")
        reverse = kind == "ddim_reverse"
        T = tables.num_timesteps
        _require_cuda(x_T, "x_T")
        if reverse:
            if noise is not None:
                raise ValueError("the reverse DDIM loop is deterministic: noise must be None")
        else:
            _require_cuda(noise, "noise")
            assert noise.shape == (T, job.n_nodes, 3)
        assert x_T.shape == (job.n_nodes, 3)
        if pin is not None:
            pin = self._pin_arrays(pin, job.n_nodes)
        if streams is None:
            streams = 2 if job.n_nodes >= self.SPLIT_MIN_NODES and len(job.sample_struct) >= 2 else 1
        if streams > 1:
            parts = job.parts(streams)
            pins = None if pin is None else [(pin[0][i], pin[1][i]) for _p, i in parts]
            noises = [None if reverse else noise[:, i] for _p, i in parts]
            outs = self.sample_many([p for p, _i in parts], [x_T[i] for _p, i in parts], noises,
                                    tables, check=check, coef=coef, pins=pins, kind=kind)
            x0 = torch.empty(job.n_nodes, 3, dtype=torch.float32, device=self.device)
            for (_p, i), o in zip(parts, outs):
                x0[i] = o
            return x0
        if coef is None:
            coef = tables.step_coefficients() if kind == "ddpm" else tables.ddim_coefficients(reverse=reverse)
        fixed_var = bool(int(coef[0, 7]) & 2)
        if self.weights.out_dim != (3 if fixed_var else 6):
            raise ValueError(f"the {kind.upper()} loop needs a model with 6 outputs (mean | variance logits), or 3 with a "
                             "fixed-variance sampler (create_diffusion(learn_sigma=False)); a flow-matching model is sampled "
                             "with codlad_amd.diffusion_and_flow.ode.odeint")
        x = x_T.detach().clone().contiguous().float()
        noise = None if reverse else noise.contiguous().float()
        mods = self.step_mods(tables.timestep_map)
        mode = int(coef[0, 7])
        coef = torch.from_numpy(coef).to(self.device)
        st = job.structures
        self._fresh_features(st)
        x_start = torch.empty_like(x) if self.self_condition else None
        if kind != "ddpm":
            rc = self.lib.codlad_ddim_loop(C.byref(self.weights.struct), _lib.ptr(job.node_info), job.n_nodes,
                                           _lib.ptr(st.E_idx), _lib.ptr(st.h_E0), _lib.ptr(st.E1), st.n_snodes,
                                           _lib.ptr(x), _lib.ptr(x_start), _lib.ptr(noise), _lib.ptr(mods),
                                           _lib.ptr(coef), T, mode, int(reverse),
                                           _lib.ptr(None if pin is None else pin[0]),
                                           _lib.ptr(None if pin is None else pin[1]), C.byref(job.ws),
                                           _lib.stream_ptr(self.device))
            _lib.check(rc, "codlad_ddim_loop")
        elif pin is None:
            rc = self.lib.codlad_sample_loop(C.byref(self.weights.struct), _lib.ptr(job.node_info),
                                             job.n_nodes, _lib.ptr(st.E_idx), _lib.ptr(st.h_E0),
                                             _lib.ptr(st.E1), st.n_snodes, _lib.ptr(x), _lib.ptr(x_start),
                                             _lib.ptr(noise), _lib.ptr(mods), _lib.ptr(coef), T, C.byref(job.ws),
                                             _lib.stream_ptr(self.device))
            _lib.check(rc, "codlad_sample_loop")
        else:
            rc = self.lib.codlad_sample_loop_pinned(C.byref(self.weights.struct), _lib.ptr(job.node_info),
                                                    job.n_nodes, _lib.ptr(st.E_idx), _lib.ptr(st.h_E0),
                                                    _lib.ptr(st.E1), st.n_snodes, _lib.ptr(x), _lib.ptr(x_start),
                                                    _lib.ptr(noise), _lib.ptr(mods), _lib.ptr(coef), T,
                                                    _lib.ptr(pin[0]), _lib.ptr(pin[1]), C.byref(job.ws),
                                                    _lib.stream_ptr(self.device))
            _lib.check(rc, "codlad_sample_loop_pinned")
        if check:
            self.check_status(job)
        return x

    def sample_many(self, jobs, x_Ts, noises, tables, check=True, coef=None, pins=None, kind="ddpm"):
        pins = [None] * len(jobs) if pins is None else list(pins)
        assert len(pins) == len(jobs)
        if not hasattr(self, "_streams"):
            self._streams = []
        while len(self._streams) < len(jobs):
            self._streams.append(torch.cuda.Stream(device=self.device))
        cur = torch.cuda.current_stream(self.device)
        for job in jobs:
            self._fresh_features(job.structures)
        self.step_mods(tables.timestep_map)
        outs = []
        for job, x_T, noise, pin, st in zip(jobs, x_Ts, noises, pins, self._streams):
            if pin is not None:
                pin = self._pin_arrays(pin, job.n_nodes)
            st.wait_stream(cur)
            with torch.cuda.stream(st):
                outs.append(self.sample(job, x_T, noise, tables, check=False, coef=coef, streams=1, pin=pin, kind=kind))
        for st in self._streams[:len(jobs)]:
            cur.wait_stream(st)
        if check:
            for job in jobs:
                self.check_status(job)
        return outs

    @staticmethod
    def _pin_arrays(pin, n_nodes):
        x0, mask = pin
        _require_cuda(x0, "pin x0")
        _require_cuda(mask, "pin mask")
        if tuple(x0.shape) != (n_nodes, 3) or tuple(mask.shape) != (n_nodes,):
            raise ValueError(f"pin: x0 must be [{n_nodes}, 3] and mask [{n_nodes}], got {tuple(x0.shape)} and {tuple(mask.shape)}")
        if not x0.is_floating_point():
            raise TypeError(f"pin: x0 must be a floating-point tensor, got {x0.dtype}")
        if mask.dtype not in (torch.bool, torch.uint8, torch.int32):
            raise TypeError(f"pin: mask must be bool, uint8 or int32, got {mask.dtype}")
        x0 = x0.contiguous().float()
        if mask.dtype != torch.uint8:
            mask = mask != 0
        return x0, mask.to(torch.uint8).contiguous()

    def ddpm_update(self, x, model_out, noise, tables, i, return_x_start=False):
        _require_cuda(x, "x")
        n = x.numel() // 3
        x = x.contiguous().float()
        out = torch.empty_like(x)
        x_start = torch.empty_like(x) if return_x_start else None
        coef = np.ascontiguousarray(tables.step_coefficients()[i])
        rc = self.lib.codlad_ddpm_update(_lib.ptr(x), _lib.ptr(model_out.contiguous().float()),
                                         _lib.ptr(noise.contiguous().float()),
                                         coef.ctypes.data_as(C.c_void_p), n, _lib.ptr(out), _lib.ptr(x_start),
                                         _lib.stream_ptr(self.device))
        _lib.check(rc, "codlad_ddpm_update")
        return (out, x_start) if return_x_start else out

    @staticmethod
    def ddpm_pred_xstart(x, model_out, coef):
        _require_cuda(x, "x")
        x = x.contiguous().float()
        out = torch.empty_like(x)
        coef = np.ascontiguousarray(coef, dtype=np.float32)
        _check_step_operands(x, model_out, coef)
        rc = _lib.lib().codlad_ddpm_pred_xstart(_lib.ptr(x), _lib.ptr(model_out.contiguous().float()),
                                                coef.ctypes.data_as(C.c_void_p), x.numel() // 3, _lib.ptr(out),
                                                _lib.stream_ptr(x.device))
        _lib.check(rc, "codlad_ddpm_pred_xstart")
        return out

    @staticmethod
    def ddpm_posterior_step(x, pred_xstart, model_out, noise, coef, grad=None, fixed_variance=0.0):
        _require_cuda(x, "x")
        x = x.contiguous().float()
        out = torch.empty_like(x)
        x_start = torch.empty_like(x)
        coef = np.ascontiguousarray(coef, dtype=np.float32)
        g = None if grad is None else grad.contiguous().float()
        _check_step_operands(x, model_out, coef, pred_xstart=pred_xstart, noise=noise, grad=g)
        rc = _lib.lib().codlad_ddpm_posterior_step(_lib.ptr(x), _lib.ptr(pred_xstart.contiguous().float()),
                                                   _lib.ptr(model_out.contiguous().float()),
                                                   _lib.ptr(noise.contiguous().float()), _lib.ptr(g),
                                                   coef.ctypes.data_as(C.c_void_p), C.c_float(fixed_variance),
                                                   x.numel() // 3, _lib.ptr(out), _lib.ptr(x_start),
                                                   _lib.stream_ptr(x.device))
        _lib.check(rc, "codlad_ddpm_posterior_step")
        return out, x_start

    @staticmethod
    def ddim_step(x, pred_xstart, noise, coef, grad=None, reverse=False):
        _require_cuda(x, "x")
        x = x.contiguous().float()
        out = torch.empty_like(x)
        x_start = torch.empty_like(x)
        coef = np.ascontiguousarray(coef, dtype=np.float32)
        if reverse != (noise is None):
            raise ValueError("the forward DDIM step takes noise, the reverse one none")
        nz = None if noise is None else noise.contiguous().float()
        g = None if grad is None else grad.contiguous().float()
        _check_step_operands(x, None, coef, pred_xstart=pred_xstart, noise=nz, grad=g)
        rc = _lib.lib().codlad_ddim_step(_lib.ptr(x), _lib.ptr(pred_xstart.contiguous().float()), _lib.ptr(nz),
                                         _lib.ptr(g), coef.ctypes.data_as(C.c_void_p), int(bool(reverse)),
                                         x.numel() // 3, _lib.ptr(out), _lib.ptr(x_start), _lib.stream_ptr(x.device))
        _lib.check(rc, "codlad_ddim_step")
        return out, x_start


def _check_step_operands(x, model_out, coef, **same_as_x):
    n = x.numel() // 3
    if x.numel() != 3 * n or n == 0:
        raise ValueError(f"x must hold [n, 3] latents, got {tuple(x.shape)}")
    if coef.shape != (8,):
        raise ValueError(f"coef must be one [8] row of the step table, got {coef.shape}")
    width = 3 if int(coef[7]) & 2 else 6
    for name, t in dict(model_out=model_out, **same_as_x).items():
        if t is None:
            continue
        _require_cuda(t, name)
        want = n * (width if name == "model_out" else 3)
        if t.numel() != want:
            raise ValueError(f"{name} holds {t.numel()} values, the step needs {want} ({n} nodes)")


class Decoder:

    def __init__(self, state_dict, device, mean3=None, std3=None, angle=False, n_codes=4096):
        self.device = torch.device(device)
        if self.device.type != "cuda":
            raise RuntimeError("codlad_amd runs on an MI355X only; no CPU path exists")
        self.lib = _lib.lib()
        if state_dict is None:
            self.weights = DecoderWeights.empty(self.device, angle, n_codes)
        else:
            self.weights = DecoderWeights(state_dict, self.device, mean3, std3)
        f = dict(dtype=torch.float32, device=self.device)
        self._unit = (torch.zeros(3, **f), torch.ones(3, **f))

    @property
    def mean(self):
        return self.weights.mean

    @property
    def std(self):
        return self.weights.std

    def vq(self, x, normalised=True):
        _require_cuda(x, "latent")
        xs = x.contiguous().float()
        n = xs.numel() // 3
        idx = torch.empty(n, dtype=torch.int64, device=self.device)
        zq = torch.empty_like(xs)
        lat = torch.empty_like(xs)
        mean, std = (self.mean, self.std) if normalised else self._unit
        cb = self.weights.codebook
        rc = self.lib.codlad_vq_lookup(_lib.ptr(xs), n, _lib.ptr(mean), _lib.ptr(std), _lib.ptr(cb),
                                       cb.shape[0], _lib.ptr(idx), _lib.ptr(zq), _lib.ptr(lat),
                                       _lib.stream_ptr(self.device))
        _lib.check(rc, "codlad_vq_lookup")
        return idx, zq, lat

    @staticmethod
    def csr_from_pairs(pairs, n_nodes):
        gtr_ij = bool((pairs[:, 0] > pairs[:, 1]).any())
        gtr_ji = bool((pairs[:, 1] > pairs[:, 0]).any())
        directed = pairs if (gtr_ij and gtr_ji) else torch.cat([pairs, pairs.flip(1)], dim=0)
        recv = directed[:, 0]
        order = torch.sort(recv, stable=True).indices
        src = directed[order, 1].to(torch.int32).contiguous()
        counts = torch.bincount(recv, minlength=n_nodes)
        ptr = torch.zeros(n_nodes + 1, dtype=torch.int32, device=pairs.device)
        ptr[1:] = torch.cumsum(counts, 0).to(torch.int32)
        return ptr, src

    def build_csr(self, cg_xyz, sample_lens, cutoff=21.0, sample_range=None, max_edges=None):
        xyz = cg_xyz.to(self.device).contiguous().float()
        M = xyz.shape[0]
        rng = self.sample_ranges(sample_lens) if sample_range is None else sample_range
        assert rng.shape == (M, 2)
        deg = torch.empty(M, dtype=torch.int32, device=self.device)
        st = _lib.stream_ptr(self.device)
        _lib.check(self.lib.codlad_cg_graph(_lib.ptr(xyz), _lib.ptr(rng), M, C.c_float(cutoff), _lib.ptr(deg),
                                            None, None, st), "codlad_cg_graph(count)")
        ptr = torch.zeros(M + 1, dtype=torch.int32, device=self.device)
        ptr[1:] = torch.cumsum(deg, 0).to(torch.int32)
        n_src = max_edges if max_edges is not None else int(ptr[-1])
        src = torch.empty(max(n_src, 1), dtype=torch.int32, device=self.device)
        _lib.check(self.lib.codlad_cg_graph(_lib.ptr(xyz), _lib.ptr(rng), M, C.c_float(cutoff), None,
                                            _lib.ptr(ptr), _lib.ptr(src), st), "codlad_cg_graph(fill)")
        return ptr, src[:n_src]

    def sample_ranges(self, sample_lens):
        M = int(sum(sample_lens))
        rng = np.empty((M, 2), dtype=np.int32)
        o = 0
        for L in sample_lens:
            rng[o:o + L, 0] = o
            rng[o:o + L, 1] = L
            o += L
        return torch.from_numpy(rng).to(self.device)

    def ic_decode(self, z_q, cg_z, cg_xyz, pairs=None, csr=None):
        _require_cuda(z_q, "z_q")
        M = z_q.shape[0]
        cg_z = cg_z.to(self.device, torch.int32).contiguous()
        lo, hi = int(cg_z.min()), int(cg_z.max())
        if lo < 0 or hi >= 25:
            raise ValueError(f"cg_z (residue types {lo}..{hi}) outside the decoder's 25-row embedding tables")
        ptr, src = csr if csr is not None else self.csr_from_pairs(pairs.to(self.device), M)
        assert ptr.numel() == M + 1 and ptr.dtype == torch.int32 and src.dtype == torch.int32
        scratch = torch.empty(M, 200, dtype=torch.float32, device=self.device)
        ic = torch.empty(M, 13, 3, dtype=torch.float32, device=self.device)
        rc = self.lib.codlad_ic_decode(C.byref(self.weights.struct), _lib.ptr(z_q.contiguous().float()),
                                       _lib.ptr(cg_z),
                                       _lib.ptr(cg_xyz.to(self.device).contiguous().float()),
                                       _lib.ptr(ptr), _lib.ptr(src), M, _lib.ptr(scratch), _lib.ptr(ic),
                                       _lib.stream_ptr(self.device))
        _lib.check(rc, "codlad_ic_decode")
        return ic

    def ic_to_xyz(self, ca_full, ic, info):
        _require_cuda(ic, "ic")
        B, L = ic.shape[0], ic.shape[1]
        orders, slot_to_out, n_atoms = info_tables(info, L, self.device)
        out = torch.empty(B, n_atoms, 3, dtype=torch.float32, device=self.device)
        rc = self.lib.codlad_ic_to_xyz(_lib.ptr(ca_full.to(self.device).contiguous().float()),
                                       _lib.ptr(ic.contiguous().float()), _lib.ptr(orders),
                                       _lib.ptr(slot_to_out), B, L, n_atoms, _lib.ptr(out),
                                       _lib.stream_ptr(self.device))
        _lib.check(rc, "codlad_ic_to_xyz")
        return out


    def ic_to_xyz_groups(self, groups, reuse=False):
        key = tuple((ca.data_ptr(), ic.data_ptr(), id(info[0]), tuple(ic.shape)) for ca, ic, info in groups)
        cache = getattr(self, "_xyz_groups", None) if reuse else None
        if cache is None or cache[0] != key:
            desc = (_lib.XyzGroup * len(groups))()
            outs, keep, row = [], [], 0
            for g, (ca, ic, info) in enumerate(groups):
                _require_cuda(ic, "ic")
                B, L = ic.shape[0], ic.shape[1]
                orders, s2o, n_atoms = info_tables(info, L, self.device)
                ca_d, ic_d = ca.to(self.device).contiguous().float(), ic.contiguous().float()
                assert ic_d.data_ptr() == ic.data_ptr() and ca_d.shape == (B, L + 2, 3)
                out = torch.empty(B, n_atoms, 3, dtype=torch.float32, device=self.device)
                d = desc[g]
                d.ca_full, d.ic, d.orders, d.slot_to_out, d.xyz_out = (ca_d.data_ptr(), ic_d.data_ptr(), orders.data_ptr(),
                                                                       s2o.data_ptr(), out.data_ptr())
                d.B, d.L, d.n_atoms, d.first_row = B, L, n_atoms, row
                row += B * L
                outs.append(out)
                keep += [ca_d, ic_d, orders, s2o]
            table = torch.frombuffer(bytearray(bytes(desc)), dtype=torch.uint8).to(self.device)
            cache = (key, table, outs, keep, row)
            if reuse:
                self._xyz_groups = cache
        _key, table, outs, _keep, rows = cache
        rc = self.lib.codlad_ic_to_xyz_groups(_lib.ptr(table), len(groups), rows, _lib.stream_ptr(self.device))
        _lib.check(rc, "codlad_ic_to_xyz_groups")
        return outs


_INFO_CACHE = {}


def info_tables(info, L, device):
    permute, atom_idx, orders = info
    key = (id(permute), id(atom_idx), id(orders), L, str(device))
    if key not in _INFO_CACHE:
        assert orders.shape == (10, L, 3), "atom_orders does not match the batch's residue count"
        n_atoms = int(permute.numel())
        slot = atom_idx.cpu()[permute.cpu()]
        assert int(slot.max()) < 14 * L and torch.unique(slot).numel() == n_atoms
        s2o = torch.full((14 * L,), -1, dtype=torch.int32)
        s2o[slot] = torch.arange(n_atoms, dtype=torch.int32)
        o32 = orders.to(torch.int32).contiguous()
        assert int(o32.min()) >= 0
        for i in range(10):
            assert int(o32[i].max()) < 4 + i, "atom_orders references an atom that is not placed yet"
        if len(_INFO_CACHE) > 256:
            _INFO_CACHE.clear()
        _INFO_CACHE[key] = (o32.to(device), s2o.to(device), n_atoms, info)
    o, s, n, _keepalive = _INFO_CACHE[key]
    return o, s, n
```

### include/codlad_hip.h

```cpp
#ifndef CODLAD_HIP_H
#define CODLAD_HIP_H

#include <stdint.h>

#ifdef __cplusplus
extern "C" {
#endif

#define CODLAD_ABI_VERSION 15
#define CODLAD_H 128
#define CODLAD_KNN 64
#define CODLAD_MODS_PER_STEP 6016
#define CODLAD_PACKED_BLOCK 16384

int codlad_abi_version(void);
const char *codlad_last_error(void);
void codlad_struct_sizes(int *out5);

void codlad_pack_block_host(const float *src_host, int ld, float scale, float *dst_host);

typedef struct {
    const float *W1e, *W2, *W3;
    const float *W11e, *W12, *W13;
    const float *W1a, *W1c;
    const float *W11a, *W11c;
    const float *Win[4], *Wout[4];
    const float *b1, *b2, *b3, *b11, *b12, *b13, *b_in , *b_out;
} codlad_enc_layer;

typedef struct {
    const float *W1e;
    const float *W2, *W3;
    const float *W1a;
    const float *W1v;
    const float *TS;
    const float *Win[4], *Wout[4];
    const float *b1, *b2, *b3, *b_in, *b_out;
} codlad_dec_layer;

typedef struct {
    const void *W1e, *W2, *W3, *W11e, *W12, *W13, *W1a, *W1c, *W11a, *W11c;
    const void *Win[4], *Wout[4];
    const float *b1, *b2, *b3, *b11, *b12, *b13, *b_in, *b_out;
    int e1, e2, e3, e11, e12, e13, e_in, e_out;
} codlad_enc_layer_h;

typedef struct {
    const void *W1e, *W2, *W3, *W1a, *W1v;
    const void *Win[4], *Wout[4];
    const float *TS;
    const float *b1, *b2, *b3, *b_in, *b_out;
    int e1, e2, e3, e_in, e_out;
} codlad_dec_layer_h;

typedef struct {
    const float *freqs;
    const float *rbf_mu;
    const float *t_w0, *t_b0;
    const float *t_w2, *t_b2;
    const float *ada_w[7], *ada_b[7];
    const float *x_in_w, *x_in_b;
    const float *pos_w, *pos_b;
    const float *edge_wT;
    const float *norm_w, *norm_b;
    const float *We_wT, *We_b;
    const float *out_w, *out_b;
    codlad_enc_layer enc[3];
    codlad_dec_layer dec[3];
    int precision;
    codlad_enc_layer_h enc_h[3];
    codlad_dec_layer_h dec_h[3];
    int self_condition;
    int out_dim;
} codlad_denoiser_weights;

int codlad_features_prepass(const codlad_denoiser_weights *w, const float *cg_xyz,
                            const int32_t *snode_info, int n_snodes, int max_len,
                            int32_t *E_idx, float *h_E0, void *stream);

int codlad_step_mods(const codlad_denoiser_weights *w, const int64_t *t_values, int n_t,
                     float *mods, void *stream);

int codlad_step_mods_f(const codlad_denoiser_weights *w, const float *t_values, int n_t, float *mods, void *stream);

int codlad_ode_combine(const float *y, const float *const *k_host, const float *coef_host, int n_k, float h,
                       size_t n, float *out, void *stream);

typedef struct {
    float *hV;
    float *hVenc;
    float *S;
    float *PQ;
    float *hE;
    int32_t *status;
    const int32_t *tile_list;
    int32_t n_tiles;
} codlad_workspace;

#define CODLAD_STATUS_NONFINITE 1
#define CODLAD_E_NONFINITE (-3)

int codlad_status_check(int32_t *status, void *stream);

int codlad_layer0_edge_terms(const codlad_denoiser_weights *w, const int32_t *snode_info,
                             int n_snodes, const float *h_E0, float *E1, void *stream);

int codlad_denoiser_forward(const codlad_denoiser_weights *w, const int32_t *node_info,
                            int n_nodes, const int32_t *E_idx, const float *h_E0,
                            const float *E1, int n_snodes, const float *x, const float *x_self_cond,
                            const float *mods_t, float *out, const codlad_workspace *ws, void *stream);

int codlad_ddpm_update(const float *x, const float *model_out, const float *noise,
                       const float *coef_host, int n_nodes, float *x_out, float *x_start_out ,
                       void *stream);

int codlad_ddpm_pred_xstart(const float *x, const float *model_out, const float *coef_host, int n_nodes,
                            float *pred_xstart, void *stream);

int codlad_ddpm_posterior_step(const float *x, const float *pred_xstart, const float *model_out, const float *noise,
                               const float *grad , const float *coef_host, float fixed_variance,
                               int n_nodes, float *x_out, float *x_start_out , void *stream);

int codlad_sample_loop(const codlad_denoiser_weights *w, const int32_t *node_info, int n_nodes,
                       const int32_t *E_idx, const float *h_E0, const float *E1, int n_snodes,
                       float *x, float *x_start, const float *noise, const float *mods, const float *coef,
                       int T, const codlad_workspace *ws, void *stream);

int codlad_sample_loop_pinned(const codlad_denoiser_weights *w, const int32_t *node_info, int n_nodes,
                              const int32_t *E_idx, const float *h_E0, const float *E1, int n_snodes,
                              float *x, float *x_start, const float *noise, const float *mods, const float *coef,
                              int T, const float *pin_x0, const uint8_t *pin_mask, const codlad_workspace *ws,
                              void *stream);

int codlad_ddim_loop(const codlad_denoiser_weights *w, const int32_t *node_info, int n_nodes, const int32_t *E_idx,
                     const float *h_E0, const float *E1, int n_snodes, float *x, float *x_start,
                     const float *noise , const float *mods, const float *coef, int T, int mode,
                     int reverse, const float *pin_x0 , const uint8_t *pin_mask ,
                     const codlad_workspace *ws, void *stream);

int codlad_ddim_step(const float *x, const float *pred_xstart, const float *noise ,
                     const float *grad , const float *coef_host, int reverse, int n_nodes, float *x_out,
                     float *x_start_out , void *stream);

int codlad_vq_lookup(const float *x, int n, const float *mean3, const float *std3,
                     const float *codebook, int n_codes, int64_t *idx, float *z_q,
                     float *latent_out , void *stream);

typedef struct {
    int angle;
    const float *map_out_w, *map_out_b;
    const float *res_embed;
    const float *inv0_w[4], *inv0_b[4], *inv1_w[4], *inv1_b[4];
    const float *dist_w[4], *dist_b[4];
    const float *dense1_w[4], *dense1_b[4], *dense3_w[4], *dense3_b[4];
    const float *bb_dist, *sc_dist;
    const float *bb_ang1_w, *bb_ang1_b, *bb_ang3_w, *bb_ang3_b;
    const float *sc_angle_emb;
    const float *sc_ang1_w, *sc_ang1_b, *sc_ang3_w, *sc_ang3_b;
    const float *bb_tor1_w, *bb_tor1_b, *bb_tor3_w, *bb_tor3_b;
    const float *tor1_w[4], *tor1_b[4], *tor3_w[4], *tor3_b[4];
    const float *fin1_w, *fin1_b, *fin3_w, *fin3_b;
} codlad_decoder_weights;

int codlad_ic_decode(const codlad_decoder_weights *w, const float *z_q, const int32_t *cg_z,
                     const float *cg_xyz, const int32_t *csr_ptr, const int32_t *csr_src,
                     int M, float *scratch, float *ic_out, void *stream);

int codlad_cg_graph(const float *cg_xyz, const int32_t *sample_range, int M, float cutoff,
                    int32_t *degree, const int32_t *csr_ptr, int32_t *csr_src, void *stream);

typedef struct {
    const int32_t *ptr, *snd;
    int32_t n_recv;
    const float *xyz_recv, *xyz_snd;
    const float *typ_recv, *typ_snd;
    float r_sign, smear_stop;
    const float *emb0_w, *emb0_b, *emb3_w, *emb3_b;
    int32_t emb_in;
    const float *h_recv; int32_t d_recv;
    const float *h_snd; int32_t d_snd;
    int32_t attr_recv_first;
    const float *fc0_w, *fc0_b, *fc3_w, *fc3_b;
    int32_t depth;
    float *out;
    int32_t accumulate, group;
    const void *packed;
} codlad_tp_conv_args;
int codlad_tp_conv(const codlad_tp_conv_args *args, void *stream);
int codlad_tp_conv_args_size(void);
int codlad_tp_conv_image_bytes(int depth);
int codlad_tp_conv_pack(const codlad_tp_conv_args *args, void *image, void *stream);

int codlad_receiver_csr(const int64_t *pairs, int n_pairs, int n_nodes, int mode, int32_t *ptr, int32_t *snd, int32_t *work,
                        void *stream);

int codlad_mlp_rows(const float *x, int n, int in_dim, const float *w1, const float *b1, int hidden, const float *w2,
                    const float *b2, int out_dim, int act, int mode, float *y, void *stream);
int codlad_bead_mean(const float *h_atom, const float *h_cg, const int32_t *bead_ptr, const int32_t *bead_atoms,
                     int n_cg, float *node, void *stream);
int codlad_embed_rows(const float *table, const int32_t *idx, int n, int width, float *out, void *stream);

int codlad_ic_to_xyz(const float *ca_full, const float *ic, const int32_t *orders,
                     const int32_t *slot_to_out, int B, int L, int n_atoms, float *xyz_out,
                     void *stream);

typedef struct {
    const float *ca_full, *ic;
    const int32_t *orders, *slot_to_out;
    float *xyz_out;
    int32_t B, L, n_atoms, first_row;
} codlad_xyz_group;
int codlad_ic_to_xyz_groups(const codlad_xyz_group *groups, int n_groups, int total_rows, void *stream);

int codlad_xyz_to_ic(const float *xyz, int n_frames, int n_atoms, const int32_t *quads, int n_quads, float *ic_out,
                     void *stream);

#define CODLAD_OPT_NODEQ_MAX_TILES 0
#define CODLAD_OPT_EDGE_TILE_MAX_NODES 1
#define CODLAD_OPT_NODE_QUAD_MAX_TILES 2
#define CODLAD_OPT_DEC_EDGE_VARIANT 3
#define CODLAD_OPT_TP_CONV_VARIANT 4
#define CODLAD_OPT_EDGE_UPD_VARIANT 5
#define CODLAD_OPT_EDGE_CUS 6
#define CODLAD_OPT_EDGE_WIDE_MAX_TILES 7
#define CODLAD_N_OPTIONS 8
int codlad_set_option(int option, int value);

int codlad_probe_edge_launches(int enable);
int codlad_probe_read(int kind, double *total_ms);

int codlad_bench_edge_launch(const codlad_denoiser_weights *w, const int32_t *node_info,
                             int n_nodes, const int32_t *E_idx, const float *h_E0,
                             const float *mods_t, const codlad_workspace *ws, int which,
                             int layer, void *stream);

typedef struct {
    const float *xyz_recon, *xyz;
    int64_t n_atoms;
    const int64_t *edge_list;
    int64_t n_edges;
    const int64_t *clash_list;
    int64_t n_clash;
    const int64_t *bb_NO_list;
    int64_t n_bb;
    const int64_t *interaction_list;
    int64_t n_inter;
    const int64_t *pi_pi_list;
    int64_t n_pipi;
    const float *ic, *ic_recon, *ic_mask;
    int64_t n_ic;
} codlad_metric_inputs;

int codlad_metrics_scratch_bytes(void);
int codlad_eval_metrics(const codlad_metric_inputs *in, float *out8, void *scratch, void *stream);

int codlad_bond_graph_counts(const float *xyz, const float *xyz_recon, const float *radius, const int32_t *heavy,
                             const int32_t *struct_ptr, int n_struct, int max_atoms, float scale, int32_t *counts,
                             void *stream);

int codlad_selftest_gemm128(const float *W_packed, const float *bias, const float *X, int n_rows,
                            int act, float *Y, void *stream);

int codlad_selftest_gemm128_h(const void *W_split, const float *bias, const float *X, int n_rows,
                              int act_in, int terms, float *Y, void *stream);

#ifdef __cplusplus
}
#endif
#endif
```

Baseline: 681.9 structures/s.

## Pack partial edge tiles of adjacent nodes and cost-balance XCD node ranges

In the edge message and edge update kernels, a node with 33-48 neighbours is paired with a following node that has at most 16 (or 33-48) neighbours, so the leftover 16-lane half tile of one node shares a 32-wide tile with the other. This removes padded MFMA work on half-empty tiles. A host planner also computes per-XCD node bounds that balance the new paired tile cost across the 8 XCD chunks, replacing the equal-node split. The kernels gain extra LDS state, more control flow and extra shuffles, and the pairing depends on the order of K values along the strided walk.

```diff
diff --git a/codlad_amd/_lib.py b/codlad_amd/_lib.py
--- a/codlad_amd/_lib.py
+++ b/codlad_amd/_lib.py
@@ -4,7 +4,7 @@
 import torch
 
 _HERE = os.path.dirname(os.path.abspath(__file__))
-ABI_VERSION = 15
+ABI_VERSION = 16
 LIB_PATH = os.environ.get("CODLAD_HIP_LIB") or os.path.join(_HERE, "libcodlad_hip.so")
 
 P = C.c_void_p
@@ -45,7 +45,7 @@
 
 
 class Workspace(C.Structure):
-    _fields_ = [(n, P) for n in ("hV", "hVenc", "S", "PQ", "hE", "status", "tile_list")] + [("n_tiles", C.c_int32)]
+    _fields_ = [(n, P) for n in ("hV", "hVenc", "S", "PQ", "hE", "status", "tile_list")] + [("n_tiles", C.c_int32), ("xcd_bounds", P)]
 
 
 class DecoderWeights(C.Structure):
@@ -100,6 +100,7 @@
                                           C.POINTER(Workspace), P]),
     "codlad_status_check": (C.c_int, [P, P]),
     "codlad_set_option": (C.c_int, [C.c_int, C.c_int]),
+    "codlad_edge_plan_host": (C.c_int, [P, C.c_int, C.c_int, C.c_int, C.c_int, P, P]),
     "codlad_ddpm_update": (C.c_int, [P, P, P, P, C.c_int, P, P, P]),
     "codlad_ddpm_pred_xstart": (C.c_int, [P, P, P, C.c_int, P, P]),
     "codlad_ddpm_posterior_step": (C.c_int, [P, P, P, P, P, P, C.c_float, C.c_int, P, P, P]),
@@ -152,6 +153,17 @@
 
 
 OPT_NODEQ_MAX_TILES, OPT_EDGE_TILE_MAX_NODES, OPT_DEC_EDGE_VARIANT, OPT_TP_CONV_VARIANT, OPT_EDGE_UPD_VARIANT, OPT_EDGE_CUS, OPT_EDGE_WIDE_MAX_TILES, OPT_NODE_QUAD_MAX_TILES = 0, 1, 3, 4, 5, 6, 7, 2
+OPT_EDGE_PAIR = 8
+EDGE_GRID = (256, 8)
+
+
+def edge_plan(K, pair=True, grid=EDGE_GRID):
+    import numpy as np
+    K = np.ascontiguousarray(K, dtype=np.int32)
+    bounds, stats = np.zeros(9, dtype=np.int32), np.zeros(20, dtype=np.int64)
+    check(lib().codlad_edge_plan_host(K.ctypes.data_as(P), K.shape[0], grid[0], grid[1], int(bool(pair)),
+                                      bounds.ctypes.data_as(P), stats.ctypes.data_as(P)), "codlad_edge_plan_host")
+    return bounds, stats
 
 
 def set_option(option, value):
diff --git a/codlad_amd/csrc/denoiser_kernels.hip b/codlad_amd/csrc/denoiser_kernels.hip
--- a/codlad_amd/csrc/denoiser_kernels.hip
+++ b/codlad_amd/csrc/denoiser_kernels.hip
@@ -3,6 +3,7 @@
 #include "../../include/codlad_hip.h"
 
 #include "edge_args.h"
+#include <vector>
 
 
 template <bool EDGE_UPDATE>
@@ -573,7 +574,7 @@
     else hipLaunchKernelGGL((node_kernel_h<false, NW, TERMS>), grid, block, lds, st, na);
 }
 
-static int g_options[CODLAD_N_OPTIONS] = {-1, -1, -1, -1, -1, -1, -1, -1};
+static int g_options[CODLAD_N_OPTIONS] = {-1, -1, -1, -1, -1, -1, -1, -1, -1};
 static int option_or(int opt, const char *env, int dflt) {
     if (g_options[opt] < 0) {
         const char *e = getenv(env);
@@ -595,6 +596,89 @@
 int edge_cus() {
     const int v = option_or(CODLAD_OPT_EDGE_CUS, "CODLAD_EDGE_CUS", 0);
     return v > 0 && v < num_cu() ? v : num_cu();
+}
+static int edge_pair() { return option_or(CODLAD_OPT_EDGE_PAIR, "CODLAD_EDGE_PAIR", 1) != 0; }
+static void set_edge_walk(EdgeArgs &ea, const codlad_workspace *ws) {
+    ea.pair = edge_pair();
+    ea.xcd_bounds = ea.pair ? ws->xcd_bounds : nullptr;
+}
+
+static int64_t chunk_walk(const int32_t *K, int lo, int hi, int stride, bool pair, int64_t *pairs) {
+    int64_t tiles = 0;
+    for (int w = 0; w < stride; ++w)
+        for (int n = lo + w; n < hi; n += stride) {
+            tiles += K[n] > 32 ? 2 : 1;
+            if (pair && n + stride < hi && edge_pair_ok(K[n], K[n + stride])) {
+                n += stride;
+                tiles += (K[n] > 32 ? 2 : 1) - 1;
+                if (pairs) ++*pairs;
+            }
+        }
+    return tiles;
+}
+
+extern "C" int codlad_edge_plan_host(const int32_t *K_host, int n_nodes, int n_workgroups, int waves_per_workgroup,
+                                     int pair, int32_t *bounds_host, int64_t *stats_host) {
+    CODLAD_REQUIRE(K_host && n_nodes > 0 && n_workgroups > 0 && waves_per_workgroup > 0, "bad arguments");
+    int32_t bounds[9];
+    const int G = XCD_BOUND_GRANULE, ng = (n_nodes + G - 1) / G;
+    std::vector<int64_t> upto(ng + 1, 0);
+    int64_t plain = 0;
+    for (int n = 0; n < n_nodes; ++n) {
+        CODLAD_REQUIRE(K_host[n] >= 1 && K_host[n] <= 64, "K outside 1..64");
+        plain += K_host[n] > 32 ? 2 : 1;
+        upto[n / G + 1] += pair ? edge_node_cost2(K_host[n]) : (K_host[n] > 32 ? 4 : 2);
+    }
+    for (int g = 0; g < ng; ++g) upto[g + 1] += upto[g];
+    const int64_t total = upto[ng];
+    const bool chunked = n_workgroups % 8 == 0;
+    const int stride = chunked ? n_workgroups / 8 * waves_per_workgroup : n_workgroups * waves_per_workgroup;
+    auto node_of = [&](int g) { return g * G < n_nodes ? g * G : n_nodes; };
+    if (pair) {
+        double target = total / 16.0;
+        for (int pass = 0; pass < (chunked ? 3 : 1); ++pass) {
+            bounds[0] = 0;
+            int g = 0;
+            int64_t done = 0;
+            for (int x = 1; x < 8; ++x) {
+                const int g0 = g;
+                if (pass == 0) {
+                    while (g < ng && 8 * upto[g + 1] <= total * x) ++g;
+                    if (g < ng && 8 * upto[g + 1] - total * x < total * x - 8 * upto[g]) ++g;
+                } else {
+                    auto f = [&](int gg) { return (double)(done + chunk_walk(K_host, node_of(g0), node_of(gg), stride, true, nullptr)); };
+                    const double want = target * x;
+                    while (g < ng && f(g) < want) ++g;
+                    while (g > g0 && f(g - 1) >= want) --g;
+                    if (g > g0 && want - f(g - 1) < f(g) - want) --g;
+                }
+                bounds[x] = node_of(g);
+                if (chunked) done += chunk_walk(K_host, node_of(g0), node_of(g), stride, true, nullptr);
+            }
+            bounds[8] = n_nodes;
+            if (chunked) target = (done + chunk_walk(K_host, bounds[7], n_nodes, stride, true, nullptr)) / 8.0;
+        }
+    } else {
+        const int chunk = xcd_chunk_nodes(n_nodes);
+        for (int x = 0; x <= 8; ++x) bounds[x] = (int64_t)x * chunk < n_nodes ? x * chunk : n_nodes;
+    }
+    if (bounds_host)
+        for (int x = 0; x <= 8; ++x) bounds_host[x] = bounds[x];
+    if (stats_host) {
+        int64_t walk = 0, pairs = 0;
+        for (int x = 0; x < 8; ++x) {
+            const int lo = (bounds[x] + G - 1) / G, hi = (bounds[x + 1] + G - 1) / G;
+            stats_host[4 + x] = upto[hi] - upto[lo];
+            stats_host[12 + x] = chunked ? chunk_walk(K_host, bounds[x], bounds[x + 1], stride, pair != 0, &pairs) : 0;
+            walk += stats_host[12 + x];
+        }
+        if (!chunked) walk = chunk_walk(K_host, 0, n_nodes, stride, pair != 0, &pairs);
+        stats_host[0] = plain;
+        stats_host[1] = total;
+        stats_host[2] = walk;
+        stats_host[3] = pairs;
+    }
+    return 0;
 }
 
 void launch_node_wide(int terms, bool upd, const NodeArgs &na, hipStream_t st);
@@ -674,6 +758,7 @@
         ea.P = PQ0; ea.Q = PQ1; ea.W1 = L.W1e; ea.W2 = L.W2; ea.S = ws->S;
         ea.W1h = Lh.W1e; ea.W2h = Lh.W2;
         set_msg_scales(ea, split, L.b2, Lh.b2, Lh.e1, Lh.e2);
+        set_edge_walk(ea, ws);
         if (l == 0 && E1) ea.E1 = E1;
         launch_edge(false, ea, w->precision, st, tile_list, ws->n_tiles);
 
@@ -713,6 +798,7 @@
         eu.mods3 = m + 6 * HD;
         eu.W1h = Lh.W11e; eu.W2h = Lh.W12; eu.W3h = Lh.W13;
         set_upd_scales(eu, split, L, Lh);
+        set_edge_walk(eu, ws);
         if (l == 0 && E1) eu.E1 = E1 + n_snodes * 64 * HD;
         launch_edge(true, eu, w->precision, st, tile_list, ws->n_tiles);
     }
@@ -725,6 +811,7 @@
         ea.P = PQ0; ea.Q = PQ1; ea.W1 = L.W1e; ea.W2 = L.W2; ea.S = ws->S;
         ea.W1h = Lh.W1e; ea.W2h = Lh.W2;
         set_msg_scales(ea, split, L.b2, Lh.b2, Lh.e1, Lh.e2);
+        set_edge_walk(ea, ws);
         launch_edge(false, ea, w->precision, st, tile_list, ws->n_tiles);
 
         NodeArgs na = {};
@@ -1028,6 +1115,7 @@
         ea.W1h = Lh.W11e; ea.W2h = Lh.W12; ea.W3h = Lh.W13;
         set_upd_scales(ea, split, L, Lh);
     }
+    set_edge_walk(ea, ws);
     launch_edge(which == 1, ea, w->precision, (hipStream_t)stream, nullptr, ws->n_tiles);
     return codlad_check_launch("codlad_bench_edge_launch");
 }
diff --git a/codlad_amd/csrc/edge_args.h b/codlad_amd/csrc/edge_args.h
--- a/codlad_amd/csrc/edge_args.h
+++ b/codlad_amd/csrc/edge_args.h
@@ -24,6 +24,8 @@
     int n_nodes;
     GeluK gelu_a, gelu_b;
     float res_scale, ln_eps;
+    const int32_t *xcd_bounds;
+    int pair;
 };
 
 struct EdgeTileArgs : EdgeArgs {
@@ -41,15 +43,33 @@
     return g * ((tiles + 7) / 8);
 }
 
+__host__ __device__ inline bool edge_node_eligible(int K) { return K <= 16 || (K > 32 && K <= 48); }
+__host__ __device__ inline bool edge_pair_ok(int K, int K_next) {
+    return K > 32 && K <= 48 && edge_node_eligible(K_next);
+}
+__host__ __device__ inline int edge_node_cost2(int K) { return K <= 32 ? 2 : (K <= 48 ? 3 : 4); }
+constexpr int XCD_BOUND_GRANULE = 32;
+
 struct NodeSpan {
     int first, end, stride;
 };
-DEV NodeSpan wave_node_span(int n_nodes, int nwaves, int wave) {
-    const int nb = gridDim.x, b = blockIdx.x;
+__host__ __device__ inline NodeSpan node_span_of(int n_nodes, int nwaves, int wave, int nb, int b, const int32_t *bounds) {
     if (nb % 8) return {b * nwaves + wave, n_nodes, nb * nwaves};
-    const int chunk = xcd_chunk_nodes(n_nodes);
-    const int lo = (b % 8) * chunk, hi = lo + chunk < n_nodes ? lo + chunk : n_nodes;
+    int lo, hi;
+    if (bounds) {
+        lo = bounds[b % 8];
+        hi = bounds[b % 8 + 1];
+    } else {
+        const int chunk = xcd_chunk_nodes(n_nodes);
+        lo = (b % 8) * chunk;
+        hi = lo + chunk;
+    }
+    if (lo > n_nodes) lo = n_nodes;
+    if (hi > n_nodes) hi = n_nodes;
     return {lo + (b / 8) * nwaves + wave, hi, (nb / 8) * nwaves};
+}
+DEV NodeSpan wave_node_span(int n_nodes, int nwaves, int wave, const int32_t *bounds = nullptr) {
+    return node_span_of(n_nodes, nwaves, wave, gridDim.x, blockIdx.x, bounds);
 }
 
 constexpr int UPD_W1_KS = 3;
diff --git a/codlad_amd/csrc/edge_msg_kernel.hip b/codlad_amd/csrc/edge_msg_kernel.hip
--- a/codlad_amd/csrc/edge_msg_kernel.hip
+++ b/codlad_amd/csrc/edge_msg_kernel.hip
@@ -1,10 +1,12 @@
 #include "edge_args.h"
+
+constexpr int MSG_PAIR_U4 = 32 + 64 + 16;
 
 template <int NWAVES, bool HOISTED, int TERMS>
 __global__ __launch_bounds__(NWAVES * 64, NWAVES / 4) void msg_kernel_h(EdgeArgs a) {
     extern __shared__ __align__(16) u32x4 wl[];
     constexpr int NT = NWAVES * 64;
-    const int tid = threadIdx.x, lane = tid & 63, wave = tid >> 6;
+    const int tid = threadIdx.x, lane = tid & 63, wave = __builtin_amdgcn_readfirstlane(tid >> 6);
     u32x4 *consts = wl + 2 * LDS_BLOCK_U4;
     {
         const u32x4 *g1 = reinterpret_cast<const u32x4 *>(a.W1h);
@@ -23,17 +25,18 @@
     __syncthreads();
     const u32x4 *w1 = wl, *w2 = wl + LDS_BLOCK_U4;
     const float *c_b2 = reinterpret_cast<const float *>(consts);
-    float2 *Pslot = reinterpret_cast<float2 *>(consts + EDGE_CONST_U4 + wave * 32);
     const int h = lane >> 5, c = lane & 31;
-    const NodeSpan span = wave_node_span(a.n_nodes, NWAVES, wave);
+    float2 *const Pslot0 = reinterpret_cast<float2 *>(consts + EDGE_CONST_U4 + wave * 32);
+    float2 *const Pslot1 = reinterpret_cast<float2 *>(consts + EDGE_CONST_U4 + NWAVES * 32 + 4 * 128 + wave * MSG_PAIR_U4);
+    float4 *wait_sum = reinterpret_cast<float4 *>(Pslot1 + 64) + lane;
+    int *wait_j = reinterpret_cast<int *>(Pslot1 + 64 + 2 * 64) + lane;
+    const NodeSpan span = wave_node_span(a.n_nodes, NWAVES, wave, a.xcd_bounds);
     const int stride = span.stride, n_end = span.end;
-    int n = span.first;
+    int n = __builtin_amdgcn_readfirstlane(span.first);
     if (n >= n_end) return;
 
     const float *xsrc = HOISTED ? a.E1 : a.hE_in;
-    auto block_of = [&](int node, int s) {
-        return xsrc + (size_t)((HOISTED || a.in_by_src) ? s : node) * EDGE_BLOCK;
-    };
+    const bool by_src = HOISTED || a.in_by_src;
     const float2 *Prows = reinterpret_cast<const float2 *>(a.P);
 
     int4 info = a.node_info[n];
@@ -41,10 +44,12 @@
     int K = __builtin_amdgcn_readfirstlane(info.z);
     int jA = a.E_idx[(size_t)src * 64 + (c < K ? c : 0)];
     int jB = a.E_idx[(size_t)src * 64 + (32 + c < K ? 32 + c : 0)];
-    Pslot[lane] = Prows[(size_t)n * 64 + lane];
+    int cs = 0;
+    Pslot0[lane] = Prows[(size_t)n * 64 + lane];
     int half = 0;
+    int ph = 0, wn = 0, wait_src = 0, wait_base = 0, wK = 0;
     Tile x, acc, t2;
-    tile_load_edge<!HOISTED>(x, block_of(n, src), c < K ? c : 0, h);
+    tile_load_edge<!HOISTED>(x, xsrc + (size_t)(by_src ? src : n) * EDGE_BLOCK, c < K ? c : 0, h);
     tile_load_row(acc, a.Q + (size_t)(base + jA) * HD, h);
     float sum[4] = {0.f, 0.f, 0.f, 0.f};
     const float4 *bias_rep = reinterpret_cast<const float4 *>(consts + EDGE_CONST_U4 + NWAVES * 32) + c;
@@ -57,7 +62,10 @@
         const bool next_node = n2 < n_end;
         const bool first_half = half == 0;
         if (first_half && next_node) ninfo = a.node_info[n2];
-        tile_add_row(acc, reinterpret_cast<const float *>(Pslot), h);
+        {
+            const float2 *pl = ((ph == 2 && c < 16) ? !cs : cs) ? Pslot1 : Pslot0;
+            tile_add_row(acc, reinterpret_cast<const float *>(pl), h);
+        }
         if (HOISTED) {
 #pragma unroll
             for (int bo = 0; bo < 4; ++bo) acc.b[bo] += x.b[bo];
@@ -72,7 +80,9 @@
             njB = a.E_idx[(size_t)nsrc * 64 + (32 + c < nK ? 32 + c : 0)];
             npv = Prows[(size_t)n2 * 64 + lane];
         }
-        const bool next_half = first_half && K > 32;
+        const bool open_pair = a.pair && ph == 0 && first_half && next_node && edge_pair_ok(K, nK);
+        const bool next_half = first_half && K > 32 && !open_pair;
+        const bool shared_next = ph == 1 || (open_pair && nK <= 32);
         {
             int rep_off = 0;
             asm volatile("" : "+v"(rep_off));
@@ -88,16 +98,55 @@
         }
         gemm128_h_lds<TERMS, true, true>(t2, acc, w2, lane, a.gelu_a);
         {
-            const int pn = next_half ? n : (next_node ? n2 : n), ps = next_half ? src : nsrc;
-            const int pe = next_half ? (32 + c < K ? 32 + c : 0) : (c < nK ? c : 0);
-            const int pq = next_half ? base + jB : nbase + njA;
-            tile_load_edge<!HOISTED>(x, block_of(pn, ps), pe, h);
+            int fn = next_half ? n : (next_node ? n2 : n), fs = next_half ? src : nsrc;
+            int fb = next_half ? base : nbase, fK = next_half ? K : nK;
+            int sn = fn, ss = fs, sb = fb, sK = fK;
+            int jl = next_half ? jB : njA, jh = jl;
+            int lo_off = next_half ? 32 : 0, hi_off = lo_off;
+            if (shared_next) {
+                if (ph == 1) {
+                    fn = wn; fs = wait_src; fb = wait_base; fK = wK;
+                    sn = n; ss = src; sb = base; sK = K;
+                    jl = *wait_j;
+                    jh = __shfl(jB, lane - 16);
+                } else {
+                    fn = n; fs = src; fb = base; fK = K;
+                    sn = n2; ss = nsrc; sb = nbase; sK = nK;
+                    jl = jB;
+                    jh = __shfl(njA, lane - 16);
+                }
+                lo_off = 32;
+                hi_off = (sK > 32 ? 32 : 0) - 16;
+            }
+            const bool low = c < 16;
+            const int want = (low ? lo_off : hi_off) + c;
+            const int pe = want < (low ? fK : sK) ? want : 0;
+            const float *fblk = xsrc + (size_t)(by_src ? fs : fn) * EDGE_BLOCK, *sblk = xsrc + (size_t)(by_src ? ss : sn) * EDGE_BLOCK;
+            const int pq = low ? fb + jl : sb + jh;
+            tile_load_edge<!HOISTED>(x, low ? fblk : sblk, pe, h);
             tile_load_row(acc, a.Q + (size_t)pq * HD, h);
             __builtin_amdgcn_sched_barrier(0);
         }
         tile_gelu(t2, a.gelu_b);
         const int cnt = K - 32 * half;
-        if (cnt >= 32) {
+        if (ph == 2) {
+            const int wcnt = wK - 32;
+            const float4 ws4 = *wait_sum;
+            const float wsum[4] = {ws4.x, ws4.y, ws4.z, ws4.w};
+#pragma unroll
+            for (int bo = 0; bo < 4; ++bo) {
+                float s0 = 0.f, s1 = 0.f;
+#pragma unroll
+                for (int r = 0; r < 8; ++r) {
+                    s0 += ((r & 3) + 8 * (r >> 2) + 4 * h < wcnt) ? t2.b[bo][r] : 0.f;
+                    s1 += ((r & 3) + 8 * (r >> 2) + 4 * h < cnt) ? t2.b[bo][8 + r] : 0.f;
+                }
+                sum[bo] += s1;
+                const float ws = wsum[bo] + s0;
+                const float tot = ws + __shfl_xor(ws, 32);
+                if (h == 0) a.S[(size_t)wn * HD + 32 * bo + c] = tot;
+            }
+        } else if (cnt >= 32) {
 #pragma unroll
             for (int bo = 0; bo < 4; ++bo) {
                 f32x2 s2 = tile_pair(t2.b[bo], 0);
@@ -116,17 +165,29 @@
         }
         if (next_half) {
             half = 1;
+            if (ph == 1) ph = 2;
             continue;
         }
-#pragma unroll
-        for (int bo = 0; bo < 4; ++bo) {
-            const float tot = sum[bo] + __shfl_xor(sum[bo], 32);
-            if (h == 0) a.S[(size_t)n * HD + 32 * bo + c] = tot;
-            sum[bo] = 0.f;
-        }
-        if (!next_node) break;
+        if (open_pair) {
+            *wait_sum = make_float4(sum[0], sum[1], sum[2], sum[3]);
+            *wait_j = jB;
+#pragma unroll
+            for (int bo = 0; bo < 4; ++bo) sum[bo] = 0.f;
+            wn = n; wait_src = src; wait_base = base; wK = K;
+            ph = nK > 32 ? 1 : 2;
+            cs ^= 1;
+        } else {
+#pragma unroll
+            for (int bo = 0; bo < 4; ++bo) {
+                const float tot = sum[bo] + __shfl_xor(sum[bo], 32);
+                if (h == 0) a.S[(size_t)n * HD + 32 * bo + c] = tot;
+                sum[bo] = 0.f;
+            }
+            if (!next_node) break;
+            ph = 0;
+        }
         n = n2; src = nsrc; base = nbase; K = nK; jA = njA; jB = njB;
-        Pslot[lane] = npv;
+        (cs ? Pslot1 : Pslot0)[lane] = npv;
         half = 0;
     }
 }
@@ -136,8 +197,8 @@
 static void launch_msg_t(const EdgeArgs &ea, hipStream_t st) {
     static bool attr_set = false;
     constexpr int NW = 8;
-    const size_t lds = 16 * (edge_lds_u4<false, NW>() + 4 * 128);
-    static_assert(16 * (edge_lds_u4<false, NW>() + 4 * 128) <= 160 * 1024, "kernel exceeds the CU's LDS");
+    const size_t lds = 16 * (edge_lds_u4<false, NW>() + 4 * 128 + NW * MSG_PAIR_U4);
+    static_assert(16 * (edge_lds_u4<false, NW>() + 4 * 128 + NW * MSG_PAIR_U4) <= 160 * 1024, "kernel exceeds the CU's LDS");
     if (!attr_set) {
         set_max_lds(reinterpret_cast<const void *>(msg_kernel_h<NW, false, TERMS>), lds);
         set_max_lds(reinterpret_cast<const void *>(msg_kernel_h<NW, true, TERMS>), lds);
diff --git a/codlad_amd/csrc/edge_upd_kernel.hip b/codlad_amd/csrc/edge_upd_kernel.hip
--- a/codlad_amd/csrc/edge_upd_kernel.hip
+++ b/codlad_amd/csrc/edge_upd_kernel.hip
@@ -5,7 +5,7 @@
     extern __shared__ __align__(16) u32x4 wl[];
     constexpr int NT = NWAVES * 64;
     constexpr int W1_U4 = UPD_W1_KS * 512;
-    const int tid = threadIdx.x, lane = tid & 63, wave = tid >> 6;
+    const int tid = threadIdx.x, lane = tid & 63, wave = __builtin_amdgcn_readfirstlane(tid >> 6);
     u32x4 *consts = wl + 2 * LDS_BLOCK_U4 + W1_U4;
     {
         const u32x4 *g1 = reinterpret_cast<const u32x4 *>(a.W1h);
@@ -33,34 +33,57 @@
     const float *c_base = reinterpret_cast<const float *>(consts);
     float *Pslot = reinterpret_cast<float *>(consts + EDGE_CONST_U4 + wave * 32);
     const int h = lane >> 5, c = lane & 31;
-    const NodeSpan span = wave_node_span(a.n_nodes, NWAVES, wave);
-    for (int n = span.first; n < span.end; n += span.stride) {
+    const NodeSpan span = wave_node_span(a.n_nodes, NWAVES, wave, a.xcd_bounds);
+    int pend_n = -1, pend_src = 0, pend_base = 0, pend_K = 0;
+    for (int nv = span.first; nv < span.end; nv += span.stride) {
+        const int n = __builtin_amdgcn_readfirstlane(nv);
         const int4 info = a.node_info[n];
-        const int src = info.x, base = info.y, K = info.z;
-        const float *rows = a.hE_in + (size_t)(a.in_by_src ? src : n) * EDGE_BLOCK;
-        float *out_rows = a.hE_out + (size_t)n * EDGE_BLOCK;
-        const bool validA = c < K, validB = 32 + c < K;
-        const int colA = validA ? c : 0, colB = validB ? 32 + c : 0;
-        const int jA = a.E_idx[(size_t)src * 64 + colA], jB = a.E_idx[(size_t)src * 64 + colB];
+        const int src = __builtin_amdgcn_readfirstlane(info.x), base = __builtin_amdgcn_readfirstlane(info.y);
+        const int K = __builtin_amdgcn_readfirstlane(info.z);
+        const int Ku = K, lh = Ku > 32;
+        const bool paired = pend_n >= 0;
+        bool open_pair = false;
+        if (a.pair && !paired && Ku > 32 && Ku <= 48 && n + span.stride < span.end)
+            open_pair = edge_pair_ok(Ku, __builtin_amdgcn_readfirstlane(a.node_info[n + span.stride].z));
+        const bool ptA = paired && !lh, ptB = paired && lh;
+        const bool lowA = ptA && c < 16, lowB = ptB && c < 16;
+        const int wantA = ptA ? (c < 16 ? 32 + c : c - 16) : c, wantB = ptB ? 32 + (c & 15) : 32 + c;
+        const bool validA = wantA < (lowA ? pend_K : K), validB = wantB < (lowB ? pend_K : K);
+        const int colA = validA ? wantA : 0, colB = validB ? wantB : 0;
+        const int jA = a.E_idx[(size_t)(lowA ? pend_src : src) * 64 + colA];
+        const int jB = a.E_idx[(size_t)(lowB ? pend_src : src) * 64 + colB];
         reinterpret_cast<float2 *>(Pslot)[lane] = reinterpret_cast<const float2 *>(a.P + (size_t)n * HD)[lane];
 
         for (int half = 0; half < 2; ++half) {
             if (32 * half >= K) break;
+            if (half && open_pair) break;
+            const bool ptile = half ? ptB : ptA, low = half ? lowB : lowA;
             const bool valid = half ? validB : validA;
-            const int colc = half ? colB : colA, col = 32 * half + c;
+            const int colc = half ? colB : colA;
             const int j = half ? jB : jA;
+            const int base_l = low ? pend_base : base;
+            const float *rows_n = a.hE_in + (size_t)(a.in_by_src ? src : n) * EDGE_BLOCK;
+            const float *rows_p = a.hE_in + (size_t)(a.in_by_src ? pend_src : pend_n) * EDGE_BLOCK;
+            const float *rows = low ? rows_p : rows_n;
+            float *out_rows = a.hE_out + (size_t)(low ? pend_n : n) * EDGE_BLOCK;
             Tile x, acc, t2;
             StreamedGemm<TERMS, UPD_W1_KS, 8 - UPD_W1_KS, false, 8, true> tail1;
+            float2 pend_p = {0.f, 0.f};
+            if (ptile) pend_p = reinterpret_cast<const float2 *>(a.P + (size_t)pend_n * HD)[lane];
             if (!HOISTED) tail1.start(a.W1h, lane);
             int lds_off = 0;
             asm volatile("" : "+v"(lds_off));
             const float *c_b2 = c_base + lds_off, *c_b3 = c_b2 + HD;
             const float *c_modA = c_b2 + 2 * HD, *c_modB = c_b2 + 3 * HD;
-            tile_load_row(acc, a.Q + (size_t)(base + j) * HD, h);
-            tile_add_row(acc, Pslot, h);
+            tile_load_row(acc, a.Q + (size_t)(base_l + j) * HD, h);
+            if (!low) tile_add_row(acc, Pslot, h);
+            if (ptile) {
+                reinterpret_cast<float2 *>(Pslot)[lane] = pend_p;
+                if (low) tile_add_row(acc, Pslot, h);
+            }
             if (!HOISTED) tile_load_edge<true>(x, rows, colc, h);
             if (HOISTED) {
-                tile_add_edge(acc, a.E1 + (size_t)src * EDGE_BLOCK, colc, h);
+                tile_add_edge(acc, low ? a.E1 + (size_t)pend_src * EDGE_BLOCK : a.E1 + (size_t)src * EDGE_BLOCK, colc, h);
                 __builtin_amdgcn_sched_barrier(0);
                 tile_load_edge<false>(x, rows, colc, h);
             } else {
@@ -73,8 +96,14 @@
             gemm128_h_lds<TERMS, true>(x, t2, w3, lane, a.gelu_b);
             tile_layernorm_affine(x, a.ln_eps, c_modA, c_modB, h);
             tile_presplit(x);
-            if (valid) tile_store_edge<true>(x, out_rows, col, h);
+            if (valid) tile_store_edge<true>(x, out_rows, colc, h);
         }
+        if (open_pair) {
+            pend_n = n;
+            pend_src = src;
+            pend_base = base;
+            pend_K = K;
+        } else pend_n = -1;
     }
 }
 
diff --git a/codlad_amd/engine.py b/codlad_amd/engine.py
--- a/codlad_amd/engine.py
+++ b/codlad_amd/engine.py
@@ -94,6 +94,8 @@
         ws.hV, ws.hVenc, ws.S, ws.PQ, ws.hE, ws.status, ws.tile_list = (
             _lib.ptr(t) for t in (self.hV, self.hVenc, self.S, self.PQ, self.hE, self.status, self.tile_list))
         ws.n_tiles = tiles.shape[0]
+        self.xcd_bounds = torch.from_numpy(_lib.edge_plan(info[:, 2])[0]).to(device)
+        ws.xcd_bounds = _lib.ptr(self.xcd_bounds)
         self.ws = ws
 
     def workspace_bytes(self):
diff --git a/include/codlad_hip.h b/include/codlad_hip.h
--- a/include/codlad_hip.h
+++ b/include/codlad_hip.h
@@ -7,7 +7,7 @@
 extern "C" {
 #endif
 
-#define CODLAD_ABI_VERSION 15
+#define CODLAD_ABI_VERSION 16
 #define CODLAD_H 128
 #define CODLAD_KNN 64
 #define CODLAD_MODS_PER_STEP 6016
@@ -95,7 +95,11 @@
     int32_t *status;
     const int32_t *tile_list;
     int32_t n_tiles;
+    const int32_t *xcd_bounds;
 } codlad_workspace;
+
+int codlad_edge_plan_host(const int32_t *K_host, int n_nodes, int n_workgroups, int waves_per_workgroup, int pair,
+                          int32_t *bounds_host, int64_t *stats_host);
 
 #define CODLAD_STATUS_NONFINITE 1
 #define CODLAD_E_NONFINITE (-3)
@@ -223,7 +227,8 @@
 #define CODLAD_OPT_EDGE_UPD_VARIANT 5
 #define CODLAD_OPT_EDGE_CUS 6
 #define CODLAD_OPT_EDGE_WIDE_MAX_TILES 7
-#define CODLAD_N_OPTIONS 8
+#define CODLAD_OPT_EDGE_PAIR 8
+#define CODLAD_N_OPTIONS 9
 int codlad_set_option(int option, int value);
 
 int codlad_probe_edge_launches(int enable);
```

Result: faster. 696.6 structures/s (median of 6 runs) (+2.2%).
